# Justin-Huber/SfM-project

Hardware: AMD Instinct MI355X
Metric: verified matches/sec (match+RANSAC) (higher is better)
Workload: dtype int8 MFMA -> exact int32 (K1), f32 (K2); 1 GPU; cfg4: all 124750 unordered pairs of 500 synthetic images x 4096 128-D u8 SIFT-like descriptors; L2 match (mutual cross check + ratio 4/5) + 8-point RANSAC 4096 hyp/pair (seed 42, Sampson 1 px^2, min 15 inliers); launches of <= 131072 pairs; n_img=500, k=4096, n_hyp=4096, pairs_total=124750, pairs_rank0=124750, launches_rank0=1, parallelism=pair-sharded dp1

## Files before the change

include/sfmcore.h:

```cpp
#ifndef SFMCORE_H
#define SFMCORE_H

#include <stdint.h>

#ifdef __cplusplus
extern "C" {
#endif

#define SFM_OK 0
#define SFM_ERR_INVALID (-1)
#define SFM_ERR_HIP (-2)
#define SFM_ERR_NOMEM (-3)

#define SFM_METRIC_L2 0
#define SFM_METRIC_HAMMING 1

#define SFM_XC_NONE 0
#define SFM_XC_MUTUAL 1
#define SFM_XC_OPENCV 2

typedef struct sfm_ctx sfm_ctx;

typedef struct sfm_match_params {
    int32_t metric;
    int32_t cross_check;
    int32_t ratio_num;
    int32_t ratio_den;
    int64_t max_dist;
} sfm_match_params;

typedef struct sfm_ransac_params {
    int32_t n_hyp;
    int32_t min_inliers;
    float thr;
    int32_t _pad;
    uint64_t seed;
} sfm_ransac_params;

int sfm_ctx_create(int32_t device, sfm_ctx** out);
int sfm_ctx_destroy(sfm_ctx* ctx);
int sfm_ctx_set_stream(sfm_ctx* ctx, void* hip_stream);
int sfm_ctx_sync(sfm_ctx* ctx);
const char* sfm_last_error(void);
int32_t sfm_version(void);

int sfm_match_batch(sfm_ctx* ctx, const uint8_t* desc, const int32_t* n_kp, int32_t n_img,
                    int32_t k_max, int32_t dim, const int32_t* pairs, int32_t n_pairs,
                    const sfm_match_params* prm, int32_t* out_count, int32_t* out_match,
                    int32_t* out_dist);
int sfm_match_batch_both(sfm_ctx* ctx, const uint8_t* desc, const int32_t* n_kp, int32_t n_img,
                         int32_t k_max, int32_t dim, const int32_t* pairs, int32_t n_pairs,
                         const sfm_match_params* prm, int32_t* out_count, int32_t* out_match,
                         int32_t* out_dist);

int sfm_ransac_f_batch(sfm_ctx* ctx, const float* kps, int32_t n_img, int32_t k_max,
                       const int32_t* pairs, int32_t n_pairs, const int32_t* match_count,
                       const int32_t* matches, const sfm_ransac_params* prm,
                       int32_t* out_inl_count, int32_t* out_best_h, uint8_t* out_mask,
                       float* out_F, float* out_norm);

int sfm_ransac_f_batch_f64(sfm_ctx* ctx, const double* kps, int32_t n_img, int32_t k_max,
                           const int32_t* pairs, int32_t n_pairs, const int32_t* match_count,
                           const int32_t* matches, const sfm_ransac_params* prm,
                           int32_t* out_inl_count, int32_t* out_best_h, uint8_t* out_mask,
                           double* out_F, double* out_norm);

int sfm_ransac_counts(sfm_ctx* ctx, const float* kps, int32_t n_img, int32_t k_max,
                      const int32_t* pairs, int32_t n_pairs, const int32_t* match_count,
                      const int32_t* matches, const sfm_ransac_params* prm, int32_t* out_counts,
                      float* out_norm, float* out_hyp_F, uint8_t* out_hyp_mask);

int sfm_ransac_stats(sfm_ctx* ctx, int32_t enable, uint64_t* out);
int sfm_ransac_wave_stops(sfm_ctx* ctx, int32_t n_pairs, int32_t n_hyp, uint32_t* out);

int sfm_ransac_h_batch(sfm_ctx* ctx, const float* kps, int32_t n_img, int32_t k_max,
                       const int32_t* pairs, int32_t n_pairs, const int32_t* match_count,
                       const int32_t* matches, const sfm_ransac_params* prm,
                       int32_t* out_inl_count, int32_t* out_best_h, uint8_t* out_mask,
                       float* out_H, float* out_norm);

int sfm_ransac_h_counts(sfm_ctx* ctx, const float* kps, int32_t n_img, int32_t k_max,
                        const int32_t* pairs, int32_t n_pairs, const int32_t* match_count,
                        const int32_t* matches, const sfm_ransac_params* prm, int32_t* out_counts,
                        float* out_norm, float* out_hyp_H);

typedef struct sfm_two_view_pose_params {
    int32_t struct_size;
    int32_t min_inliers;
    float wide_key;
} sfm_two_view_pose_params;
int sfm_two_view_pose_batch(sfm_ctx* ctx, const float* kps, int32_t n_img, int32_t k_max,
                            const int32_t* pairs, int32_t n_pairs, const int32_t* match_count,
                            const int32_t* matches, const uint8_t* mask,
                            const int32_t* inl_count, const double* intr,
                            const sfm_two_view_pose_params* prm, double* out_E, double* out_R,
                            double* out_t, int32_t* out_stat, float* out_median_key);

int sfm_graph_offsets(sfm_ctx* ctx, int32_t n_pairs, const int32_t* inl_count,
                      int32_t min_inliers, int64_t* out_offsets);
int sfm_graph_rows(sfm_ctx* ctx, int32_t n_pairs, int32_t k_max, int32_t pair_base,
                   const int32_t* match_count, const int32_t* matches, const uint8_t* mask,
                   const int32_t* inl_count, int32_t min_inliers, const int64_t* offsets,
                   int32_t* out_rows);
int sfm_graph_rows_packed(sfm_ctx* ctx, int32_t n_pairs, int32_t k_max,
                          const int32_t* match_count, const int32_t* matches, const uint8_t* mask,
                          const int32_t* inl_count, int32_t min_inliers, const int64_t* offsets,
                          uint32_t* out_packed);
int sfm_graph_expand(sfm_ctx* ctx, int32_t n_pairs, int32_t pair_base, const int32_t* counts,
                     const int64_t* src_offsets, const int64_t* dst_offsets,
                     const uint32_t* packed, int32_t* out_rows);

int sfm_ba_jtj(sfm_ctx* ctx, int32_t n_cam, const double* cams, const double* pp, int32_t n_pt,
               const double* pts, int32_t n_obs, const int32_t* cam_idx, const int32_t* pt_idx,
               const double* uv, const int32_t* pt_ptr, const int32_t* cam_ptr,
               const int32_t* cam_obs, double loss_s, double* U, double* V, double* W,
               double* gc, double* gp, double* res, double* cost);

typedef struct sfm_ba_solve_params {
    double lambda;
    double tol;
    int32_t max_iter;
    int32_t poll;
    int32_t poll_first;
} sfm_ba_solve_params;
#define SFM_BA_POLL_DEFAULT 8

int sfm_ba_solve(sfm_ctx* ctx, int32_t n_cam, int32_t n_pt, int32_t n_obs,
                 const int32_t* cam_idx, const int32_t* pt_idx, const int32_t* pt_ptr,
                 const int32_t* cam_ptr, const int32_t* cam_obs, const double* U, const double* V,
                 const double* W, const double* gc, const double* gp,
                 const sfm_ba_solve_params* prm, double* dc, double* dp, double* info);
#define SFM_BA_STAGE_SETUP 0
#define SFM_BA_STAGE_SETUP_FINISH 1
#define SFM_BA_STAGE_ITER 2
#define SFM_BA_STAGE_ITER_FINISH 3
#define SFM_BA_STAGE_BACKSUB 4
#define SFM_BA_STAGE_MODEL 5
#define SFM_BA_STAGE_POLL 6
#define SFM_BA_STAGE_SCHUR 7
int sfm_ba_solve_stage(sfm_ctx* ctx, int32_t stage, int32_t k, int32_t n_cam, int32_t n_pt,
                       int32_t n_obs, const int32_t* cam_idx, const int32_t* pt_idx,
                       const int32_t* pt_ptr, const int32_t* cam_ptr, const int32_t* cam_obs,
                       const double* U, const double* V, const double* W, const double* gc,
                       const double* gp, const sfm_ba_solve_params* prm, double* comm, double* dc,
                       double* dp, double* info, int32_t* done);
int sfm_ba_fix_params(sfm_ctx* ctx, int32_t n_cam, int32_t n_obs, const int32_t* cam_idx,
                      const uint8_t* fixed, double* U, double* W, double* gc);
int sfm_ba_cost(sfm_ctx* ctx, int32_t n_cam, const double* cams, const double* pp, int32_t n_pt,
                const double* pts, int32_t n_obs, const int32_t* cam_idx, const int32_t* pt_idx,
                const double* uv, double loss_s, double* cost);
int sfm_ba_update(sfm_ctx* ctx, int32_t n_cam, const double* cams, const double* dc, int32_t n_pt,
                  const double* pts, const double* dp, double* cams_out, double* pts_out);

#define SFM_BA_MAX_CHUNKS 16
int sfm_ba_set_chunks(sfm_ctx* ctx, int32_t n_chunk, const int32_t* chunk_pt,
                      const int32_t* chunk_obs, int32_t n_total, const int32_t* cam_bounds);
int sfm_ba_chunk_tree(sfm_ctx* ctx, int32_t n_total, int64_t n, const double* parts, double* out);

int sfm_ba_set_schur(sfm_ctx* ctx, int32_t n_slot, const int32_t* slot_cam, int32_t n_seg,
                     const int32_t* seg, int32_t n_inst, const int32_t* inst, const int32_t* row_ptr,
                     int32_t n_ent, const int32_t* row_ent, int32_t n_group, const int32_t* sg_ptr,
                     const int32_t* sg, const int32_t* gk);

int sfm_tracks(sfm_ctx* ctx, int32_t n_img, const int32_t* img_base, int32_t n_pairs,
               const int32_t* pairs, int64_t n_rows, const int32_t* rows, int32_t min_len,
               int32_t* out_n_tracks, int32_t* out_track_ptr, int32_t* out_track_img,
               int32_t* out_track_kp);

int sfm_triangulate(sfm_ctx* ctx, int32_t n_cam, const double* cams, const double* pp,
                    int32_t n_pt, const int32_t* pt_ptr, const int32_t* cam_idx, const double* uv,
                    double* out_pts, double* out_stats);

typedef struct sfm_register_params {
    int32_t n_hyp;
    int32_t refine;
    double thr;
    uint64_t seed;
} sfm_register_params;

int sfm_register_batch(sfm_ctx* ctx, int32_t n_img, const int32_t* corr_ptr, const double* xy,
                       const double* X, const double* intr, const int32_t* img_id,
                       const sfm_register_params* prm, double* out_cams, int32_t* out_count,
                       int32_t* out_key, uint8_t* out_mask);

typedef struct sfm_orb_params {
    int32_t n_features;
    int32_t n_levels;
    double scale_factor;
    int32_t fast_threshold;
    int32_t _pad;
} sfm_orb_params;

int sfm_orb_batch(sfm_ctx* ctx, const uint8_t* images, int32_t n_img, int32_t H, int32_t W,
                  const sfm_orb_params* prm, float* out_kp, uint8_t* out_desc,
                  int32_t* out_count);

int sfm_calib_mfma_i8(sfm_ctx* ctx, float target_ms, double* out);

int sfm_match_cert_stats(sfm_ctx* ctx, int32_t enable, uint64_t* out);

#ifdef __cplusplus
}
#endif
#endif
```

sfm-project_amd/csrc/match_l2fr.hip:

```cpp
#include <algorithm>
#include <climits>
#include <cstdlib>

#include "l2fr_records.h"
#include "match_common.h"

namespace {

typedef int v4i __attribute__((ext_vector_type(4)));
typedef int v16i __attribute__((ext_vector_type(16)));
typedef __attribute__((address_space(3))) void lds_void;
typedef const __attribute__((address_space(1))) void gbl_void;

constexpr int D = 128;
#ifndef L2FR_WAVES
#define L2FR_WAVES 8
#endif
constexpr int WAVES = L2FR_WAVES;
constexpr int SCAN_THREADS = 64 * WAVES;
#ifndef L2FR_QT
#define L2FR_QT 4
#endif
constexpr int QT = L2FR_QT;
constexpr int QB = WAVES * QT * 32;
constexpr int SCAN_MIN_WAVES = 8 / QT;
#ifndef L2FR_CHUNK
#define L2FR_CHUNK 256
#endif
constexpr int CHUNK = L2FR_CHUNK;
constexpr int GROUP = 256;
constexpr int NT = CHUNK / 32;
constexpr int NK = D / 32;
constexpr int SLOTS = D / 16;
constexpr int PIECES = CHUNK * D / 1024 / WAVES;
constexpr int RPP = 1024 / D;
constexpr int KALIGN = CHUNK > GROUP ? CHUNK : GROUP;
constexpr int KMAX = 4096;
constexpr int PAD_INIT = -(1 << 30);
constexpr int E_VALID = l2fr::E_NONE;
static_assert(D == l2fr::REC_D && KMAX == l2fr::REC_KMAX, "l2fr_records.h is sized for D and KMAX");
typedef unsigned long long rec8;

enum : unsigned char { ST_DROP = 0, ST_CAND = 1, ST_SLOW = 2, ST_PASS = 3 };

__device__ __forceinline__ int swz(int row) { return (row >> 1) & 7; }

__device__ __forceinline__ void top2_insert(int& tb, int& ts, int x, int y) {
    const int med = max(min(tb, x), min(max(tb, x), y));
#ifndef L2FR_NO_ASM_MAX3
    int top;
    asm("v_max3_i32 %0, %1, %2, %3" : "=v"(top) : "v"(tb), "v"(x), "v"(y), "v"(med));
#else
    const int top = max(max(x, y), tb);
#endif
    ts = max(ts, med);
    tb = top;
}

__device__ __forceinline__ int dot128(const uint4* x, const uint4* y) {
    int s = 0;
#pragma unroll
    for (int k = 0; k < 8; ++k) {
        const uint4 u = x[k], v = y[k];
        s = __builtin_amdgcn_sdot4((int)u.x, (int)v.x, s, false);
        s = __builtin_amdgcn_sdot4((int)u.y, (int)v.y, s, false);
        s = __builtin_amdgcn_sdot4((int)u.z, (int)v.z, s, false);
        s = __builtin_amdgcn_sdot4((int)u.w, (int)v.w, s, false);
    }
    return s;
}

__device__ __forceinline__ void prep_one(int img, int j, const uint8_t* __restrict__ desc,
                                         const int32_t* __restrict__ n_kp, int k_max, int k_pad,
                                         int32_t* __restrict__ norm, int32_t* __restrict__ cinit,
                                         uint8_t* __restrict__ zero_row,
                                         uint4* __restrict__ desc_i8) {
    if (img == 0 && j < D) zero_row[j] = 0;
    if (j >= k_pad) return;
    int nv = 0;
    if (j < k_max) {
        const uint4* p = (const uint4*)(desc + ((size_t)img * k_max + j) * D);
        uint4* o8 = desc_i8 + ((size_t)img * k_max + j) * SLOTS;
#pragma unroll
        for (int q = 0; q < SLOTS; ++q) {
            const uint4 v = p[q];
            const uint4 x = make_uint4(v.x ^ 0x80808080u, v.y ^ 0x80808080u, v.z ^ 0x80808080u,
                                       v.w ^ 0x80808080u);
            o8[q] = x;
            nv = __builtin_amdgcn_sdot4((int)x.x, (int)x.x, nv, false);
            nv = __builtin_amdgcn_sdot4((int)x.y, (int)x.y, nv, false);
            nv = __builtin_amdgcn_sdot4((int)x.z, (int)x.z, nv, false);
            nv = __builtin_amdgcn_sdot4((int)x.w, (int)x.w, nv, false);
        }
    }
    const size_t o = (size_t)img * k_pad + j;
    norm[o] = nv;
    cinit[o] = (j < n_kp[img]) ? -((nv + 1) >> 1) : PAD_INIT;
}

constexpr int REC_R = 4;

#ifndef L2FR_UNIT
#define L2FR_UNIT 2
#endif
constexpr int UNIT = L2FR_UNIT;
__device__ void build_units(const int32_t* __restrict__ pairs, int n_pairs, int n_img,
                            const int32_t* __restrict__ n_kp, int4* __restrict__ uinfo,
                            int32_t* __restrict__ n_units, int* lds) {
    int* cur = lds;
    int* fu = lds + n_img;
    int* ru = lds + 2 * n_img + 1;
    __shared__ int ftot;
    const int tid = threadIdx.x;
    for (int i = tid; i < n_img; i += 1024) cur[i] = 0;
    __syncthreads();
    auto live = [&](int a, int b) { return n_kp[a] > 0 && n_kp[b] > 0; };
    for (int p = tid; p < n_pairs; p += 1024)
        if (live(pairs[2 * p], pairs[2 * p + 1])) atomicAdd(&cur[pairs[2 * p]], 1);
    __syncthreads();
    if (tid == 0) {
        int f = 0, r = 0;
        for (int i = 0; i < n_img; ++i) {
            const int c = cur[i];
            fu[i] = f;
            ru[i] = r;
            f += c / UNIT;
            r += (c % UNIT) != 0;
            cur[i] = 0;
        }
        fu[n_img] = f;
        ru[n_img] = r;
        ftot = f;
        *n_units = f + r;
    }
    __syncthreads();
    for (int t = tid; t < ru[n_img] * UNIT; t += 1024) uinfo[(size_t)ftot * UNIT + t] = make_int4(-1, 0, 0, 0);
    __syncthreads();
    for (int p = tid; p < n_pairs; p += 1024) {
        const int a = pairs[2 * p], b = pairs[2 * p + 1];
        if (!live(a, b)) continue;
        const int k = atomicAdd(&cur[a], 1);
        const int nf = UNIT * (fu[a + 1] - fu[a]);
        const int u = k < nf ? fu[a] + k / UNIT : ftot + ru[a];
        const int jj = k < nf ? k % UNIT : k - nf;
        uinfo[(size_t)u * UNIT + jj] = jj ? make_int4(p, b, n_kp[b], 0)
                                          : make_int4(p, a, b, n_kp[a] | (n_kp[b] << 16));
    }
}

__device__ void order_block(int ob, const int32_t* __restrict__ pairs, int n_pairs, int n_img,
                            int32_t* __restrict__ order_f, int32_t* __restrict__ order_r,
                            int2* __restrict__ rng, int32_t* __restrict__ n_rng,
                            const int32_t* __restrict__ n_kp, int4* __restrict__ rinfo,
                            int4* __restrict__ sinfo_f, int unit_blk, int4* __restrict__ uinfo,
                            int32_t* __restrict__ n_units, int* hist) {
    if (ob == unit_blk) {
        build_units(pairs, n_pairs, n_img, n_kp, uinfo, n_units, hist);
        return;
    }
    const int tid = threadIdx.x, col = ob == 0 ? 1 : 0;
    int32_t* order = ob == 0 ? order_f : order_r;
    for (int i = tid; i < n_img; i += 1024) hist[i] = 0;
    __syncthreads();
    for (int p = tid; p < n_pairs; p += 1024) atomicAdd(&hist[pairs[2 * p + col]], 1);
    __syncthreads();
    int* roff = hist + n_img;
    if (tid == 0) {
        int off = 0, nr = 0;
        for (int i = 0; i < n_img; ++i) {
            const int c = hist[i];
            roff[i] = nr;
            nr += (c + REC_R - 1) / REC_R;
            hist[i] = off;
            off += c;
        }
        if (ob == 0) *n_rng = nr;
    }
    __syncthreads();
    if (ob == 0)
        for (int i = tid; i < n_img; i += 1024) {
            const int c = (i + 1 < n_img ? hist[i + 1] : n_pairs) - hist[i];
            for (int k = 0; k < c; k += REC_R)
                rng[roff[i] + k / REC_R] = make_int2(hist[i] + k, min(REC_R, c - k));
        }
    __syncthreads();
    __syncthreads();
    for (int p = tid; p < n_pairs; p += 1024) {
        const int a = pairs[2 * p], b = pairs[2 * p + 1];
        const int slot = atomicAdd(&hist[col ? b : a], 1);
        order[slot] = p;
        if (ob == 0) sinfo_f[slot] = make_int4(p, a, b, n_kp[a] | (n_kp[b] << 16));
    }
    if (ob != 0) return;
    __threadfence_block();
    __syncthreads();
    const int nr = *n_rng;
    for (int r = tid; r < nr; r += 1024) {
        const int2 g = rng[r];
#pragma unroll
        for (int e = 0; e < REC_R; ++e) {
            int4 v = make_int4(-1, 0, 0, 0);
            if (e < g.y) {
                const int p = order[g.x + e], a = pairs[2 * p], b = pairs[2 * p + 1];
                v = make_int4(p, a, b, n_kp[a] | (n_kp[b] << 16));
            }
            rinfo[(size_t)r * REC_R + e] = v;
        }
    }
}

__global__ __launch_bounds__(1024) void l2fr_setup_kernel(
    int n_prep, int bpi, const uint8_t* __restrict__ desc, const int32_t* __restrict__ n_kp,
    int k_max, int k_pad, int32_t* __restrict__ norm, int32_t* __restrict__ cinit,
    uint8_t* __restrict__ zero_row, uint4* __restrict__ desc_i8, const int32_t* __restrict__ pairs,
    int n_pairs, int n_img, int32_t* __restrict__ order_f, int32_t* __restrict__ order_r,
    int2* __restrict__ rng, int32_t* __restrict__ n_rng, int4* __restrict__ rinfo,
    int4* __restrict__ sinfo_f, int unit_blk, int4* __restrict__ uinfo,
    int32_t* __restrict__ n_units) {
    extern __shared__ int hist[];
    const int b = (int)blockIdx.x;
    if (b < n_prep) {
        const int img = b / bpi;
        prep_one(img, (b - img * bpi) * 1024 + (int)threadIdx.x, desc, n_kp, k_max, k_pad, norm,
                 cinit, zero_row, desc_i8);
        return;
    }
    order_block(b - n_prep, pairs, n_pairs, n_img, order_f, order_r, rng, n_rng, n_kp, rinfo,
                sinfo_f, unit_blk, uinfo, n_units, hist);
}

__device__ __forceinline__ unsigned char classify(int e1, int e2, long long A, int rnum, int rden,
                                                  long long max_dist) {
    const long long d1lo = max(A - 2LL * e1 - 1, 0LL);
    const long long d2hi = e2 > E_VALID ? A - 2LL * e2 : sfm::DIST_INF;
    if (!sfm::ratio_ok(d1lo, d2hi, rnum, rden, true) || (max_dist >= 0 && !(d1lo < max_dist)))
        return ST_DROP;
    return (e2 == e1) ? ST_SLOW : ST_CAND;
}

struct FwdCls {
    const int32_t* norm;
    int rnum, rden;
    long long max_dist;
    rec8* fwd;
    uint8_t* cls;
};

#ifdef L2FR_CLOCK
constexpr int L2FR_CLOCK_SLOTS = 1 << 16;
constexpr int L2FR_CLOCK_W = 24;
__device__ unsigned long long g_l2fr_clock[L2FR_CLOCK_W * L2FR_CLOCK_SLOTS];
#define L2FR_STAMP(i, v) \
    if (!REV && tid == 0 && blockIdx.x < L2FR_CLOCK_SLOTS) g_l2fr_clock[L2FR_CLOCK_W * (size_t)blockIdx.x + (i)] = (v)
#else
#define L2FR_STAMP(i, v)
#endif

template <bool REV>
__global__ __launch_bounds__(SCAN_THREADS, SCAN_MIN_WAVES) void l2fr_scan_kernel(
    const uint8_t* __restrict__ desc, const int32_t* __restrict__ n_kp, int k_max, int k_pad,
    const int32_t* __restrict__ cinit, const uint8_t* __restrict__ zero_row,
    const int32_t* __restrict__ pairs, int n_qblk, const int32_t* __restrict__ pair_order,
    const int4* __restrict__ sinfo, int n_blk, const int4* __restrict__ qlist,
    const int32_t* __restrict__ qcount, int4* __restrict__ out, FwdCls fc,
    const int32_t* __restrict__ n_units) {
    __shared__ __attribute__((aligned(16))) unsigned char lds0[CHUNK * D + CHUNK * 4];
    __shared__ __attribute__((aligned(16))) unsigned char lds1[CHUNK * D + CHUNK * 4];

    int p, qi, ti, nq, nb, qb;
    int p2 = -1, ti2 = 0, nb2 = 0;
    int pos = 0, kk = 0;
    if (!REV && n_units) {
        const int nu = *n_units;
        const int u8 = (nu + 7) >> 3;
        const int l = (int)(blockIdx.x >> 3);
        qb = u8 > 0 ? l / u8 : n_qblk;
        pos = (l - qb * u8) * 8 + (int)(blockIdx.x & 7);
        if (qb >= n_qblk || pos >= nu) return;
        const int4 u = sinfo[(size_t)UNIT * pos];
        asm volatile("" : : "s"(u.x), "s"(u.y), "s"(u.z), "s"(u.w));
        p = u.x;
        qi = u.y;
        ti = u.z;
        nq = u.w & 0xFFFF;
        nb = u.w >> 16;
    } else {
        const int ppx = (int)(gridDim.x >> 3) / n_qblk;
        const int l = (int)(blockIdx.x >> 3);
        const int pos = (int)(blockIdx.x & 7) * ppx + l % ppx;
        qb = l / ppx;
        if (pos >= n_blk) return;
        if (REV) {
            p = pair_order[pos];
            qi = pairs[2 * p + 1];
            ti = pairs[2 * p];
            nq = qcount[p];
            nb = n_kp[ti];
        } else {
            const int4 u = sinfo[pos];
            asm volatile("" : : "s"(u.x), "s"(u.y), "s"(u.z), "s"(u.w));
            p = u.x;
            qi = u.y;
            ti = u.z;
            nq = u.w & 0xFFFF;
            nb = u.w >> 16;
        }
    }
    if (qb * QB >= nq || nb <= 0) return;
    const int tid = threadIdx.x, wave = tid >> 6, lane = tid & 63, h = lane >> 5, r32 = lane & 31;
    L2FR_STAMP(0, __builtin_amdgcn_s_memrealtime());

    const uint8_t* db = desc + (size_t)ti * k_max * D;
    const int32_t* cib = cinit + (size_t)ti * k_pad;
    int n_chunk = (nb + CHUNK - 1) / CHUNK;
    const uint8_t* db2 = desc;
    const int32_t* cib2 = cinit;
    auto find_next = [&]() {
        p2 = -1;
        if (REV || !n_units || ++kk >= UNIT) return;
        const int4 v = sinfo[(size_t)UNIT * pos + kk];
        p2 = v.x;
        ti2 = v.y;
        nb2 = v.z;
        db2 = desc + (size_t)ti2 * k_max * D;
        cib2 = cinit + (size_t)ti2 * k_pad;
    };
    find_next();

    auto stage = [&](const uint8_t* sdb, const int32_t* scib, int snb, int ch, unsigned char* dst) {
#pragma unroll
        for (int i = 0; i < PIECES; ++i) {
            const int piece = wave * PIECES + i;
            const int row = piece * RPP + lane / SLOTS;
            const int slot = (lane % SLOTS) ^ swz(row);
            const int j = ch * CHUNK + row;
            const uint8_t* src = (j < snb) ? sdb + (size_t)j * D + slot * 16 : zero_row + slot * 16;
            __builtin_amdgcn_global_load_lds((gbl_void*)src, (lds_void*)(dst + piece * 1024), 16, 0, 0);
        }
        if (tid < CHUNK / 4) {
            const int32_t* src = scib + ch * CHUNK + tid * 4;
            __builtin_amdgcn_global_load_lds((gbl_void*)src, (lds_void*)(dst + CHUNK * D + wave * 1024),
                                             16, 0, 0);
        }
    };
    auto stage_next = [&](int ch, unsigned char* dst) {
        if (ch + 1 < n_chunk) stage(db, cib, nb, ch + 1, dst);
        else if (p2 >= 0) stage(db2, cib2, nb2, 0, dst);
    };

    const int qbase = qb * QB + wave * QT * 32;
    const bool active = qbase < nq;
    const uint8_t* da = desc + (size_t)qi * k_max * D;

    auto emit = [&](int e, int e1, int e2, int t) {
        if (REV) {
            out[(size_t)p * k_pad + e] = make_int4(e1, e2, t, 0);
        } else {
            fc.fwd[(size_t)p * k_pad + e] = l2fr::pack_fwd(e1, e2, t);
            const unsigned char st =
                classify(e1, e2, fc.norm[(size_t)qi * k_pad + e], fc.rnum, fc.rden, fc.max_dist);
            fc.cls[(size_t)p * k_pad + e] =
                st == ST_CAND ? (uint8_t)t : (st == ST_SLOW ? l2fr::CLS_SLOW : l2fr::CLS_DROP);
        }
    };

#if L2FR_MFMA16
    constexpr int QS = 2 * QT;
    const int g4 = lane >> 4, r16 = lane & 15;
    v4i bq[QS][2];
    int tb[QS], ts[QS], t1[QS];
#pragma unroll
    for (int c = 0; c < QS; ++c) {
        const int e = qbase + c * 16 + r16;
        int row = -1;
        if (e < nq) row = REV ? qlist[(size_t)p * k_pad + e].y : e;
        const v4i* src = (const v4i*)((row >= 0) ? da + (size_t)row * D + 32 * g4 : zero_row + 32 * g4);
        bq[c][0] = src[0];
        bq[c][1] = src[1];
        tb[c] = INT_MIN; ts[c] = INT_MIN; t1[c] = 0;
    }
    v4i acc[QS][2];
    auto process = [&](int ch, const unsigned char* cur, unsigned char* nxt) __attribute__((always_inline)) {
        stage_next(ch, nxt);
        const int nt = min(NT, (nb - ch * CHUNK + 31) >> 5);
        if (active) {
            const int* Ci = (const int*)(cur + CHUNK * D);
            auto load_tile = [&](int tt, v4i (&af)[2][2], v4i (&init)[2]) {
#pragma unroll
                for (int u = 0; u < 2; ++u) {
                    const int row = tt * 32 + 16 * u + r16;
                    const int sw = swz(row);
#pragma unroll
                    for (int s = 0; s < 2; ++s)
#ifdef L2FR_ABL_NOLDS
                        af[u][s] = bq[(tt + u + s) & (QS - 1)][s];
#else
                        af[u][s] = *(const v4i*)(cur + row * D + (((2 * g4 + s) ^ sw) << 4));
#endif
#ifdef L2FR_ABL_NOLDS
                    init[u] = v4i{tt, u, tt, u};
#else
                    init[u] = *(const v4i*)(Ci + tt * 32 + 16 * u + 4 * g4);
#endif
                }
            };
            v4i af[2][2], init[2];
            load_tile(0, af, init);
            for (int tt = 0; tt < nt; ++tt) {
                const int gt = ch * NT + tt;
#ifndef L2FR_NO_MPRIO
                __builtin_amdgcn_s_setprio(1);
#endif
#pragma unroll
                for (int s = 0; s < 2; ++s)
#pragma unroll
                    for (int u = 0; u < 2; ++u)
#pragma unroll
                        for (int c = 0; c < QS; ++c)
                            acc[c][u] = __builtin_amdgcn_mfma_i32_16x16x64_i8(
                                af[u][s], bq[c][s], s == 0 ? init[u] : acc[c][u], 0, 0, 0);
#ifndef L2FR_NO_MPRIO
                __builtin_amdgcn_s_setprio(0);
#endif
                if (tt + 1 < nt) load_tile(tt + 1, af, init);
#pragma unroll
                for (int c = 0; c < QS; ++c) {
                    const int o = tb[c];
#ifdef L2FR_ABL_NOEPI
                    tb[c] = max(tb[c], acc[c][0][0] ^ acc[c][1][3]);
#else
#pragma unroll
                    for (int u = 0; u < 2; ++u) {
                        top2_insert(tb[c], ts[c], acc[c][u][0], acc[c][u][1]);
                        top2_insert(tb[c], ts[c], acc[c][u][2], acc[c][u][3]);
                    }
#endif
                    t1[c] = (tb[c] != o) ? gt : t1[c];
                }
            }
        }
    };
#else
    v4i bq[QT][NK];
    int tb[QT], ts[QT], t1[QT];
#pragma unroll
    for (int c = 0; c < QT; ++c) {
        const int e = qbase + c * 32 + r32;
        int row = -1;
        if (e < nq) row = REV ? qlist[(size_t)p * k_pad + e].y : e;
        const v4i* src = (const v4i*)((row >= 0) ? da + (size_t)row * D + (D / 2) * h
                                                 : zero_row + (D / 2) * h);
#pragma unroll
        for (int s = 0; s < NK; ++s) bq[c][s] = src[s];
        tb[c] = INT_MIN; ts[c] = INT_MIN; t1[c] = 0;
    }

    v16i acc[QT];
    auto epi_all = [&](int gt) {
#pragma unroll
        for (int u = 0; u < QT; ++u) {
            const int o = tb[u];
#ifdef L2FR_ABL_NOEPI
            tb[u] = max(tb[u], acc[u][0] ^ acc[u][15]);
#else
#pragma unroll
            for (int r = 0; r < 16; r += 2) top2_insert(tb[u], ts[u], acc[u][r], acc[u][r + 1]);
#endif
            t1[u] = (tb[u] != o) ? gt : t1[u];
        }
    };

    auto process = [&](int ch, const unsigned char* cur, unsigned char* nxt) __attribute__((always_inline)) {
        stage_next(ch, nxt);
        const int nt = min(NT, (nb - ch * CHUNK + 31) >> 5);
        if (active) {
            const int* Ci = (const int*)(cur + CHUNK * D);
            auto load_tile = [&](int tt, v4i (&af)[NK], v16i& init) {
                const int row = tt * 32 + r32;
                const int sw = swz(row);
#pragma unroll
                for (int s = 0; s < NK; ++s)
#ifdef L2FR_ABL_NOLDS
                    af[s] = bq[(tt + s) & (QT - 1)][s];
#else
                    af[s] = *(const v4i*)(cur + row * D + ((((SLOTS / 2) * h + s) ^ sw) << 4));
#endif
#pragma unroll
                for (int g = 0; g < 4; ++g) {
#ifdef L2FR_ABL_NOLDS
                    const v4i cv = v4i{tt, g, tt, g};
#else
                    const v4i cv = *(const v4i*)(Ci + tt * 32 + 8 * g + 4 * h);
#endif
                    init[4 * g + 0] = cv.x; init[4 * g + 1] = cv.y;
                    init[4 * g + 2] = cv.z; init[4 * g + 3] = cv.w;
                }
            };
            v4i af[NK];
            v16i init;
            load_tile(0, af, init);
            for (int tt = 0; tt < nt; ++tt) {
                const int gt = ch * NT + tt;
#ifndef L2FR_NO_MPRIO
                __builtin_amdgcn_s_setprio(1);
#endif
#pragma unroll
                for (int s = 0; s < NK; ++s)
#pragma unroll
                    for (int c = 0; c < QT; ++c)
                        acc[c] = __builtin_amdgcn_mfma_i32_32x32x32_i8(af[s], bq[c][s],
                                                                        s == 0 ? init : acc[c], 0, 0, 0);
#ifndef L2FR_NO_MPRIO
                __builtin_amdgcn_s_setprio(0);
#endif
                if (tt + 1 < nt) load_tile(tt + 1, af, init);
                epi_all(gt);
            }
        }
    };
#endif

    auto epilogue = [&]() {
#if L2FR_MFMA16
#pragma unroll
        for (int c = 0; c < QS; ++c) {
            int e1 = tb[c], e2 = ts[c], t = t1[c];
#pragma unroll
            for (int m = 16; m <= 32; m <<= 1) {
                const int P1 = __shfl_xor(e1, m), P2 = __shfl_xor(e2, m), PT = __shfl_xor(t, m);
                e2 = max(min(e1, P1), max(e2, P2));
                t = e1 > P1 ? t : (P1 > e1 ? PT : min(t, PT));
                e1 = max(e1, P1);
            }
            const int e = qbase + c * 16 + r16;
            if (g4 == 0 && e < nq) emit(e, e1, e2, t);
            tb[c] = INT_MIN; ts[c] = INT_MIN; t1[c] = 0;
        }
#else
#pragma unroll
        for (int c = 0; c < QT; ++c) {
            const int P1 = __shfl_xor(tb[c], 32), P2 = __shfl_xor(ts[c], 32),
                      PT = __shfl_xor(t1[c], 32);
            const int e1 = max(tb[c], P1);
            const int e2 = max(min(tb[c], P1), max(ts[c], P2));
            const int t = tb[c] > P1 ? t1[c] : (P1 > tb[c] ? PT : min(t1[c], PT));
            const int e = qbase + c * 32 + r32;
            if (h == 0 && e < nq) emit(e, e1, e2, t);
            tb[c] = INT_MIN; ts[c] = INT_MIN; t1[c] = 0;
        }
#endif
    };

    if (n_chunk > 0) stage(db, cib, nb, 0, lds0);
    __syncthreads();
    L2FR_STAMP(1, __builtin_amdgcn_s_memrealtime());
    L2FR_STAMP(2, __builtin_amdgcn_s_memtime());
    auto run_pair = [&](unsigned char* s0, unsigned char* s1) __attribute__((always_inline)) {
        for (int ch = 0; ch < n_chunk; ch += 2) {
            process(ch, s0, s1);
            __syncthreads();
            if (ch < 16) L2FR_STAMP(3 + ch, __builtin_amdgcn_s_memrealtime());
            if (ch + 1 < n_chunk) process(ch + 1, s1, s0);
            __syncthreads();
            if (ch + 1 < 16) L2FR_STAMP(4 + ch, __builtin_amdgcn_s_memrealtime());
        }
    };
    int g = 0;
    for (;;) {
        if (g & 1)
            run_pair(lds1, lds0);
        else
            run_pair(lds0, lds1);
        g += n_chunk;
        L2FR_STAMP(19, __builtin_amdgcn_s_memtime());
        L2FR_STAMP(20, __builtin_amdgcn_s_memrealtime());
        if (active) epilogue();
        if (p2 < 0) break;
        p = p2;
        ti = ti2;
        nb = nb2;
        db = db2;
        cib = cib2;
        n_chunk = (nb + CHUNK - 1) / CHUNK;
        find_next();
    }
#ifdef L2FR_CLOCK
    L2FR_STAMP(21, __builtin_amdgcn_s_memrealtime());
    L2FR_STAMP(22, (unsigned)__builtin_amdgcn_s_getreg((31 << 11) | 4));
    L2FR_STAMP(23, (unsigned)__builtin_amdgcn_s_getreg((15 << 11) | 20));
#endif
}

struct Top2 { long long b1; int j1; long long b2; };

__device__ __forceinline__ Top2 top2_merge(Top2 x, Top2 y) {
    const bool xf = (x.b1 < y.b1) || (x.b1 == y.b1 && x.j1 < y.j1);
    Top2 r;
    r.b1 = xf ? x.b1 : y.b1;
    r.j1 = xf ? x.j1 : y.j1;
    r.b2 = min(min(x.b2, y.b2), xf ? y.b1 : x.b1);
    return r;
}

__device__ Top2 exact_row_scan(const uint4* qrow, const uint8_t* db, const int32_t* normb, int nb,
                               int qnorm, Top2* red) {
    const int tid = threadIdx.x;
    uint4 x[SLOTS];
#pragma unroll
    for (int s = 0; s < SLOTS; ++s) x[s] = qrow[s];
    Top2 m{sfm::DIST_INF, INT_MAX, sfm::DIST_INF};
    for (int j = tid; j < nb; j += 256) {
        const int dot = dot128(x, (const uint4*)(db + (size_t)j * D));
        const long long d = (long long)qnorm + normb[j] - 2LL * dot;
        m = top2_merge(m, Top2{d, j, sfm::DIST_INF});
    }
    red[tid] = m;
    __syncthreads();
    for (int s = 128; s > 0; s >>= 1) {
        if (tid < s) red[tid] = top2_merge(red[tid], red[tid + s]);
        __syncthreads();
    }
    const Top2 r = red[0];
    __syncthreads();
    return r;
}

__device__ __forceinline__ int compact_rec(bool keep, int4 rec, int base, int* wsum, int4* dst) {
    const int tid = threadIdx.x, lane = tid & 63, wave = tid >> 6;
    const unsigned long long bal = __ballot(keep);
    const int pre = __popcll(bal & ((1ull << lane) - 1ull));
    if (lane == 0) wsum[wave] = __popcll(bal);
    __syncthreads();
    int off = 0, tot = 0;
    for (int w = 0; w < 4; ++w) {
        const int s = wsum[w];
        off += (w < wave) ? s : 0;
        tot += s;
    }
    if (keep) dst[base + off + pre] = rec;
    __syncthreads();
    return base + tot;
}

#ifndef L2FR_REC_SB
#define L2FR_REC_SB 2
#endif
constexpr int REC_SB = L2FR_REC_SB;
__global__ __launch_bounds__(256, REC_SB > 2 ? 2 : 3) void l2fr_recover_mfma_kernel(
    const uint8_t* __restrict__ desc, int k_max, int k_pad, const int32_t* __restrict__ norm,
    const int32_t* __restrict__ cinit, const int4* __restrict__ rinfo,
    const int32_t* __restrict__ n_rng, const rec8* __restrict__ fwd,
    const uint8_t* __restrict__ cls, int rnum, int rden, long long max_dist,
    rec8* __restrict__ qst) {
    __shared__ unsigned short clist[REC_R * KMAX];
    __shared__ __attribute__((aligned(16))) int gini[GROUP];
    __shared__ unsigned char gpar[GROUP];
    __shared__ unsigned long long wlo[4], whi[4];
    __shared__ int toff[9];
    const int ngrp = k_pad / GROUP;
    const int ri = (int)(blockIdx.x / ngrp), grp = (int)(blockIdx.x % ngrp), tid = threadIdx.x;
    if (ri >= *n_rng) return;
    const int wave = tid >> 6, lane = tid & 63, h = lane >> 5, r32 = lane & 31;
    int4 pi[REC_R];
#pragma unroll
    for (int e = 0; e < REC_R; ++e) pi[e] = rinfo[(size_t)ri * REC_R + e];
    const int b = pi[0].z, nb = pi[0].w >> 16;
    const int ntiles = (nb + 31) >> 5, tg = grp * 8;
    if (nb <= 0 || tg >= ntiles) return;
    const uint8_t* db = desc + (size_t)b * k_max * D;

    uint4 cv[REC_R];
#pragma unroll
    for (int e = 0; e < REC_R; ++e) {
        cv[e] = make_uint4(0xFFFFFFFFu, 0xFFFFFFFFu, 0xFFFFFFFFu, 0xFFFFFFFFu);
        if (pi[e].x >= 0 && tid * 16 < (pi[e].w & 0xFFFF))
            cv[e] = ((const uint4*)(cls + (size_t)pi[e].x * k_pad))[tid];
    }
    v4i af[2][NK];
#pragma unroll
    for (int u = 0; u < 2; ++u) {
        const int row = (tg + 2 * wave + u) * 32 + r32;
#pragma unroll
        for (int s = 0; s < NK; ++s)
            af[u][s] = row < nb ? *(const v4i*)(db + (size_t)row * D + 64 * h + 16 * s) : v4i{0, 0, 0, 0};
    }
    {
        const size_t o = (size_t)b * k_pad + tg * 32 + tid;
        gini[tid] = cinit[o];
        gpar[tid] = (unsigned char)(norm[o] & 1);
    }
    unsigned msk[REC_R];
    unsigned long long lo = 0, hi = 0;
    const unsigned g8 = 0x01010101u * ((unsigned)grp << 3);
#pragma unroll
    for (int e = 0; e < REC_R; ++e) {
        const int na = pi[e].x >= 0 ? (pi[e].w & 0xFFFF) : 0;
        const unsigned cw[4] = {cv[e].x, cv[e].y, cv[e].z, cv[e].w};
        unsigned m = 0;
#pragma unroll
        for (int k = 0; k < 4; ++k) {
            const unsigned t = (cw[k] ^ g8) & 0xF8F8F8F8u;
            const unsigned nz = ((t & 0x7F7F7F7Fu) + 0x7F7F7F7Fu) | t;
            const unsigned z = ~nz & 0x80808080u;
            m |= (((z >> 7) & 1u) | ((z >> 14) & 2u) | ((z >> 21) & 4u) | ((z >> 28) & 8u)) << (4 * k);
        }
        const int lim = na - tid * 16;
        m &= lim >= 16 ? 0xFFFFu : (lim <= 0 ? 0u : (1u << lim) - 1u);
        msk[e] = m;
        for (unsigned mm = m; mm; mm &= mm - 1) {
            const int k = __builtin_ctz(mm);
            const unsigned c = (cw[k >> 2] >> (8 * (k & 3))) & 7u;
            const unsigned long long one = 1ull << (16 * (c & 3));
            if (c & 4) hi += one; else lo += one;
        }
    }
    unsigned long long plo = lo, phi = hi;
#pragma unroll
    for (int d = 1; d < 64; d <<= 1) {
        const unsigned long long vl = __shfl_up(plo, d), vh = __shfl_up(phi, d);
        if (lane >= d) { plo += vl; phi += vh; }
    }
    if (lane == 63) { wlo[wave] = plo; whi[wave] = phi; }
    __syncthreads();
    unsigned long long blo = 0, bhi = 0, tlo = 0, thi = 0;
#pragma unroll
    for (int w = 0; w < 4; ++w) {
        blo += w < wave ? wlo[w] : 0ull;
        bhi += w < wave ? whi[w] : 0ull;
        tlo += wlo[w];
        thi += whi[w];
    }
    unsigned long long slo = 0, shi = 0;
    {
        int o = 0;
#pragma unroll
        for (int t = 0; t < 8; ++t) {
            const unsigned long long tot = t < 4 ? tlo : thi, bef = t < 4 ? blo : bhi,
                                     mine = t < 4 ? plo - lo : phi - hi;
            const int sh = 16 * (t & 3);
            const unsigned long long v =
                (unsigned long long)(o + (int)((bef >> sh) & 0xFFFF) + (int)((mine >> sh) & 0xFFFF)) << sh;
            if (t < 4) slo |= v; else shi |= v;
            if (tid == 0) toff[t] = o;
            o += (int)((tot >> sh) & 0xFFFF);
        }
        if (tid == 0) toff[8] = o;
    }
#pragma unroll
    for (int e = 0; e < REC_R; ++e) {
        const unsigned cw[4] = {cv[e].x, cv[e].y, cv[e].z, cv[e].w};
        for (unsigned mm = msk[e]; mm; mm &= mm - 1) {
            const int k = __builtin_ctz(mm);
            const unsigned c = (cw[k >> 2] >> (8 * (k & 3))) & 7u;
            const int sh = 16 * (c & 3);
            const unsigned long long cur = (c & 4) ? shi : slo, inc = 1ull << sh;
            clist[(int)((cur >> sh) & 0xFFFF)] = (unsigned short)((e << 12) | (tid * 16 + k));
            if (c & 4) shi += inc; else slo += inc;
        }
    }
    __syncthreads();
    const int w0 = toff[2 * wave], w1 = toff[2 * wave + 2];
    const int t0 = tg + 2 * wave;
    for (int c0 = w0; c0 < w1; c0 += 32 * REC_SB) {
        v4i bf[REC_SB][NK];
        rec8 rc[REC_SB];
        int ce[REC_SB], AA[REC_SB];
#pragma unroll
        for (int k = 0; k < REC_SB; ++k) {
            const int c = c0 + 32 * k + r32;
            ce[k] = -1;
            if (c < w1) {
                const int en = clist[c], e = en >> 12, q = en & 0xFFF;
                int p = pi[0].x, a = pi[0].y;
#pragma unroll
                for (int f = 1; f < REC_R; ++f) {
                    p = e == f ? pi[f].x : p;
                    a = e == f ? pi[f].y : a;
                }
                const uint8_t* xr = desc + ((size_t)a * k_max + q) * D + 64 * h;
#pragma unroll
                for (int s = 0; s < NK; ++s) bf[k][s] = *(const v4i*)(xr + 16 * s);
                rc[k] = fwd[(size_t)p * k_pad + q];
                AA[k] = norm[(size_t)a * k_pad + q];
                ce[k] = en;
            } else {
#pragma unroll
                for (int s = 0; s < NK; ++s) bf[k][s] = v4i{0, 0, 0, 0};
                rc[k] = 0;
            }
        }
#pragma unroll
        for (int k = 0; k < REC_SB; ++k) {
            if (c0 + 32 * k >= w1) break;
            const l2fr::Fwd r = l2fr::unpack_fwd(rc[k]);
            const int mine = r.tile - t0;
            int hit = -1;
#pragma unroll
            for (int u = 0; u < 2; ++u) {
                v16i acc;
                const int* gi = gini + (2 * wave + u) * 32 + 4 * h;
#pragma unroll
                for (int g = 0; g < 4; ++g) {
                    const v4i c4 = *(const v4i*)(gi + 8 * g);
                    acc[4 * g + 0] = c4.x; acc[4 * g + 1] = c4.y;
                    acc[4 * g + 2] = c4.z; acc[4 * g + 3] = c4.w;
                }
#pragma unroll
                for (int s = 0; s < NK; ++s)
                    acc = __builtin_amdgcn_mfma_i32_32x32x32_i8(af[u][s], bf[k][s], acc, 0, 0, 0);
#pragma unroll
                for (int rr = 0; rr < 16; ++rr)
                    hit = (mine == u && acc[rr] == r.e1) ? 8 * (rr >> 2) + 4 * h + (rr & 3) : hit;
            }
            hit = max(hit, __shfl_xor(hit, 32));
            if (h == 0 && ce[k] >= 0) {
                const int e = ce[k] >> 12;
                int p = pi[0].x;
#pragma unroll
                for (int f = 1; f < REC_R; ++f) p = e == f ? pi[f].x : p;
                rec8* qs = qst + (size_t)p * k_pad + (ce[k] & 0xFFF);
                if (hit < 0) {
                    *qs = l2fr::pack_res(ST_SLOW, 0, 0, 0);
                } else {
                    const int jg = (2 * wave + mine) * 32 + hit;
                    const long long A = AA[k];
                    const long long d1 = A - 2LL * r.e1 - gpar[jg];
                    const long long d2lo = r.e2 > E_VALID ? A - 2LL * r.e2 - 1 : sfm::DIST_INF;
                    const long long d2hi = r.e2 > E_VALID ? A - 2LL * r.e2 : sfm::DIST_INF;
                    int st;
                    if (max_dist >= 0 && !(d1 < max_dist)) st = ST_DROP;
                    else if (sfm::ratio_ok(d1, d2lo, rnum, rden, true)) st = ST_PASS;
                    else if (!sfm::ratio_ok(d1, d2hi, rnum, rden, true)) st = ST_DROP;
                    else st = ST_SLOW;
                    *qs = l2fr::pack_res(st, tg * 32 + jg, (int)d1, 1);
                }
            }
        }
    }
}

__global__ __launch_bounds__(256) void l2fr_compact_kernel(
    const uint8_t* __restrict__ desc, const int32_t* __restrict__ n_kp, int k_max, int k_pad,
    const int32_t* __restrict__ norm, const int32_t* __restrict__ pairs,
    const uint8_t* __restrict__ cls, rec8* __restrict__ qst, int rnum, int rden, long long max_dist,
    int4* __restrict__ surv, int32_t* __restrict__ scount, int32_t* __restrict__ smax,
    int32_t* __restrict__ out_count, int32_t* __restrict__ out_match,
    int32_t* __restrict__ out_dist) {
    __shared__ Top2 red[256];
    __shared__ int slow[256];
    __shared__ int nslow, wsum[8], wmax[4];
    const int p = blockIdx.x, tid = threadIdx.x;
    const int a = pairs[2 * p], b = pairs[2 * p + 1];
    const int na = n_kp[a], nb = n_kp[b];
    const bool direct = out_count != nullptr;
    int32_t* om = direct ? out_match + (size_t)p * k_max * 2 : nullptr;
    int32_t* od = direct ? out_dist + (size_t)p * k_max : nullptr;
    if (na <= 0 || nb <= 0) {
        if (tid == 0) {
            if (direct) out_count[p] = 0;
            else scount[p] = 0;
        }
        return;
    }
    rec8* qs = qst + (size_t)p * k_pad;
    const uint8_t* cl = cls + (size_t)p * k_pad;
    const int32_t* na_norm = norm + (size_t)a * k_pad;
    const int32_t* nb_norm = norm + (size_t)b * k_pad;
    const uint4* qa = (const uint4*)(desc + (size_t)a * k_max * D);
    const uint8_t* db = desc + (size_t)b * k_max * D;
    int4* sv = surv + (size_t)p * k_pad;
    int base = 0, dmax = 0;
    for (int q0 = 0; q0 < na; q0 += 256) {
        const int q = q0 + tid;
        int4 r = make_int4(ST_DROP, 0, 0, 0);
        if (q < na) {
            const unsigned char c = cl[q];
            const rec8 raw = qs[q];
            if (c == l2fr::CLS_SLOW) {
                r.x = ST_SLOW;
            } else if (c != l2fr::CLS_DROP) {
                const l2fr::Res u = l2fr::unpack_res(raw);
                r = make_int4(u.st, u.j1, u.d1, u.exact);
            }
        }
        if (tid == 0) nslow = 0;
        __syncthreads();
        if (r.x == ST_SLOW) slow[atomicAdd(&nslow, 1)] = tid;
        __syncthreads();
        const int ns = nslow;
        for (int i = 0; i < ns; ++i) {
            const int who = slow[i], qq = q0 + who;
            const Top2 e = exact_row_scan(qa + (size_t)qq * SLOTS, db, nb_norm, nb, na_norm[qq], red);
            if (tid == who) {
                bool keep = sfm::ratio_ok(e.b1, e.b2, rnum, rden, true);
                keep = keep && (max_dist < 0 || e.b1 < max_dist);
                r = make_int4(keep ? ST_PASS : ST_DROP, e.j1, (int)e.b1, 1);
                if (!direct) qs[qq] = l2fr::pack_res(r.x, r.y, r.z, 1);
            }
        }
        const bool keep = r.x == ST_PASS;
        dmax = keep ? max(dmax, r.z) : dmax;
        if (direct)
            base = sfm::compact256(keep, q, r.y, r.z, base, wsum, om, od);
        else
            base = compact_rec(keep, make_int4(q, r.y, r.z, 0), base, wsum, sv);
    }
    if (tid == 0) {
        if (direct) out_count[p] = base;
        else scount[p] = base;
    }
    if (direct) return;
#pragma unroll
    for (int m = 32; m > 0; m >>= 1) dmax = max(dmax, __shfl_xor(dmax, m));
    if ((tid & 63) == 0) wmax[tid >> 6] = dmax;
    __syncthreads();
    if (tid == 0) smax[p] = max(max(wmax[0], wmax[1]), max(wmax[2], wmax[3]));
}

constexpr int CERT_TMAX = 2048;
constexpr long long CERT_CAP_DEFAULT = 16384;

__global__ __launch_bounds__(256) void l2fr_mutual_cert_kernel(
    const uint8_t* __restrict__ desc, const int32_t* __restrict__ n_kp, int k_max, int k_pad,
    const int32_t* __restrict__ norm, const int32_t* __restrict__ pairs,
    const rec8* __restrict__ fwd, const uint8_t* __restrict__ cls, const rec8* __restrict__ qst,
    const int4* __restrict__ surv, const int32_t* __restrict__ scount,
    const int32_t* __restrict__ smax, long long cap, int32_t* __restrict__ rcount,
    uint8_t* __restrict__ flag, unsigned long long* __restrict__ stats,
    int32_t* __restrict__ out_count, int32_t* __restrict__ out_match,
    int32_t* __restrict__ out_dist) {
    __shared__ unsigned long long owner[KMAX];
    __shared__ int tbound[CERT_TMAX];
    __shared__ unsigned short tq[CERT_TMAX];
    __shared__ unsigned char killed[KMAX];
    __shared__ int wsum[8];
    __shared__ int nthreat;
    const int p = blockIdx.x, tid = threadIdx.x;
    const int a = pairs[2 * p], b = pairs[2 * p + 1];
    const int na = n_kp[a], nb = n_kp[b];
    const int S = (na > 0 && nb > 0) ? scount[p] : 0;
    if (cap <= 0) {
        if (tid == 0) {
            rcount[p] = S;
            flag[p] = 1;
            if (stats) atomicAdd(&stats[1], 1ull);
        }
        return;
    }
    if (S == 0) {
        if (tid == 0) {
            rcount[p] = 0;
            flag[p] = 0;
            out_count[p] = 0;
            if (stats) atomicAdd(&stats[0], 1ull);
        }
        return;
    }
    const rec8* fw = fwd + (size_t)p * k_pad;
    const rec8* qs = qst + (size_t)p * k_pad;
    const uint8_t* cl = cls + (size_t)p * k_pad;
    const int4* sv = surv + (size_t)p * k_pad;
    const int32_t* na_norm = norm + (size_t)a * k_pad;
    const int32_t* nb_norm = norm + (size_t)b * k_pad;
    const uint4* qa = (const uint4*)(desc + (size_t)a * k_max * D);
    const uint4* dbv = (const uint4*)(desc + (size_t)b * k_max * D);

    const long long T = smax[p];
    for (int k = tid; k < S; k += 256) killed[k] = 0;
    for (int j = tid; j < nb; j += 256) owner[j] = ~0ull;
    if (tid == 0) nthreat = 0;
    __syncthreads();

    for (int q = tid; q < na; q += 256) {
        const unsigned char c = cl[q];
        const rec8 raw = qs[q];
        l2fr::Res r{ST_DROP, 0, 0, 0};
        if (c != l2fr::CLS_DROP) r = l2fr::unpack_res(raw);
        const l2fr::Fwd f = l2fr::unpack_fwd(fw[q]);
        const long long A = na_norm[q];
        long long bound;
        if (r.exact == 1) {
            if ((unsigned)r.j1 < (unsigned)nb)
                atomicMin(&owner[r.j1], ((unsigned long long)(unsigned)r.d1 << 32) | (unsigned)q);
            bound = f.e2 > E_VALID ? A - 2LL * f.e2 - 1 : sfm::DIST_INF;
        } else {
            bound = A - 2LL * f.e1 - 1;
        }
        if (bound <= T) {
            const int i = atomicAdd(&nthreat, 1);
            if (i < CERT_TMAX) {
                tq[i] = (unsigned short)q;
                tbound[i] = (int)bound;
            }
        }
    }
    __syncthreads();
    const int nT = nthreat;
    if (nT > CERT_TMAX || (long long)nT * S > cap) {
        if (tid == 0) {
            rcount[p] = S;
            flag[p] = 1;
            if (stats) atomicAdd(&stats[1], 1ull);
        }
        return;
    }
    unsigned dots = 0;
    for (int i = tid; i < nT * S; i += 256) {
        const int t = i / S, k = i - t * S;
        const int4 s = sv[k];
        const int qp = tq[t];
        if (qp == s.x || s.z < tbound[t]) continue;
        const int dot = dot128(qa + (size_t)qp * SLOTS, dbv + (size_t)s.y * SLOTS);
        const long long d = (long long)na_norm[qp] + nb_norm[s.y] - 2LL * dot;
        if (d < s.z || (d == s.z && qp < s.x)) killed[k] = 1;
        ++dots;
    }
    if (stats && dots) atomicAdd(&stats[2], (unsigned long long)dots);
    __syncthreads();
    int32_t* om = out_match + (size_t)p * k_max * 2;
    int32_t* od = out_dist + (size_t)p * k_max;
    int base = 0;
    for (int k0 = 0; k0 < S; k0 += 256) {
        const int k = k0 + tid;
        int4 s = make_int4(0, 0, 0, 0);
        bool keep = false;
        if (k < S) {
            s = sv[k];
            keep = !killed[k] &&
                   owner[s.y] == (((unsigned long long)(unsigned)s.z << 32) | (unsigned)s.x);
        }
        base = sfm::compact256(keep, s.x, s.y, s.z, base, wsum, om, od);
    }
    if (tid == 0) {
        out_count[p] = base;
        rcount[p] = 0;
        flag[p] = 0;
        if (stats) atomicAdd(&stats[0], 1ull);
    }
}

__global__ __launch_bounds__(256) void l2fr_final_kernel(
    const uint8_t* __restrict__ desc, const int32_t* __restrict__ n_kp, int k_max, int k_pad,
    const int32_t* __restrict__ norm, const int32_t* __restrict__ cinit,
    const int32_t* __restrict__ pairs, const int4* __restrict__ surv,
    const int32_t* __restrict__ scount, const int4* __restrict__ rev, int mutual,
    const uint8_t* __restrict__ flag, int32_t* __restrict__ out_count,
    int32_t* __restrict__ out_match, int32_t* __restrict__ out_dist) {
    __shared__ int wsum[8];
    __shared__ int amb[256];
    __shared__ int namb;
    __shared__ unsigned char keepx[256];
    __shared__ long long redd[256];
    __shared__ int redq[256];
    const int p = blockIdx.x, tid = threadIdx.x;
    if (flag && !flag[p]) return;
    const int a = pairs[2 * p], b = pairs[2 * p + 1];
    const int na = n_kp[a], nb = n_kp[b];
    const int S = (na > 0 && nb > 0) ? scount[p] : 0;
    const int4* sv = surv + (size_t)p * k_pad;
    const int4* rv = rev + (size_t)p * k_pad;
    const int32_t* na_norm = norm + (size_t)a * k_pad;
    const int32_t* nb_norm = norm + (size_t)b * k_pad;
    const int32_t* ca = cinit + (size_t)a * k_pad;
    const uint8_t* da = desc + (size_t)a * k_max * D;
    const uint4* dbv = (const uint4*)(desc + (size_t)b * k_max * D);
    int32_t* om = out_match + (size_t)p * k_max * 2;
    int32_t* od = out_dist + (size_t)p * k_max;
    int base = 0;
    for (int k0 = 0; k0 < S; k0 += 256) {
        const int k = k0 + tid;
        int4 s = make_int4(0, 0, 0, 0);
        bool keep = false;
        if (tid == 0) namb = 0;
        __syncthreads();
        if (k < S) {
            s = sv[k];
            keep = true;
            if (mutual) {
                const int4 r = rv[k];
                const int dot = (int)(((long long)na_norm[s.x] + nb_norm[s.y] - s.z) >> 1);
                const int ep = dot + ca[s.x];
                keep = (ep == r.x) && (r.y < r.x);
                if (ep == r.x && r.y == r.x) amb[atomicAdd(&namb, 1)] = tid;
            }
        }
        keepx[tid] = keep;
        __syncthreads();
        const int nam = namb;
        for (int i = 0; i < nam; ++i) {
            const int who = amb[i];
            const int4 e = sv[k0 + who];
            uint4 y[SLOTS];
#pragma unroll
            for (int u = 0; u < SLOTS; ++u) y[u] = dbv[(size_t)e.y * SLOTS + u];
            long long bd = sfm::DIST_INF;
            int bq = INT_MAX;
            for (int q = tid; q < na; q += 256) {
                const int dot = dot128((const uint4*)(da + (size_t)q * D), y);
                const long long d = (long long)na_norm[q] + nb_norm[e.y] - 2LL * dot;
                if (d < bd) { bd = d; bq = q; }
            }
            redd[tid] = bd; redq[tid] = bq;
            __syncthreads();
            for (int st = 128; st > 0; st >>= 1) {
                if (tid < st) {
                    const long long od2 = redd[tid + st];
                    const int oq = redq[tid + st];
                    if (od2 < redd[tid] || (od2 == redd[tid] && oq < redq[tid])) {
                        redd[tid] = od2; redq[tid] = oq;
                    }
                }
                __syncthreads();
            }
            if (tid == 0) keepx[who] = (redq[0] == e.x);
            __syncthreads();
        }
        keep = keepx[tid] != 0 && k < S;
        base = sfm::compact256(keep, s.x, s.y, s.z, base, wsum, om, od);
    }
    if (tid == 0) out_count[p] = base;
}

__global__ void l2fr_dump_kernel(const int32_t* __restrict__ n_kp, const int32_t* __restrict__ pairs,
                                 int k_max, int k_pad, const int4* __restrict__ rec,
                                 const rec8* __restrict__ fwd8,
                                 const int32_t* __restrict__ cnt, int32_t* __restrict__ out_count,
                                 int32_t* __restrict__ out_match, int32_t* __restrict__ out_dist) {
    const int p = blockIdx.x;
    const int n = cnt ? cnt[p] : n_kp[pairs[2 * p]];
    for (int i = threadIdx.x; i < n; i += blockDim.x) {
        int4 r;
        if (rec) {
            r = rec[(size_t)p * k_pad + i];
        } else {
            const l2fr::Fwd f = l2fr::unpack_fwd(fwd8[(size_t)p * k_pad + i]);
            r = make_int4(f.e1, f.e2, f.tile, 0);
        }
        out_match[((size_t)p * k_max + i) * 2] = r.x;
        out_match[((size_t)p * k_max + i) * 2 + 1] = r.y;
        out_dist[(size_t)p * k_max + i] = r.z;
    }
    if (threadIdx.x == 0) out_count[p] = n;
}

}

int sfm_match_l2fr_launch(sfm_ctx* ctx, const uint8_t* desc, const int32_t* n_kp, int32_t n_img,
                          int32_t k_max, const int32_t* pairs, int32_t n_pairs,
                          const sfm_match_params* prm, int32_t* out_count, int32_t* out_match,
                          int32_t* out_dist) {
    hipStream_t st = ctx->stream;
    if (k_max == 0) {
        SFM_HIP_CHECK(hipMemsetAsync(out_count, 0, sizeof(int32_t) * n_pairs, st));
        return SFM_OK;
    }
    const int k_pad = (int)sfm::align_up((size_t)k_max, KALIGN);
    SFM_REQUIRE(k_pad <= KMAX, "sfm_match_batch: L2 matcher needs k_max <= 4096");
    const int n_qblk = (k_max + QB - 1) / QB;
    const size_t tab = (size_t)n_img * k_pad * sizeof(int32_t);
    const size_t recb = (size_t)n_pairs * k_pad * sizeof(int4);
    const size_t cntb = sfm::align_up(sizeof(int32_t) * (size_t)n_pairs, 256);
    const size_t descb = sfm::align_up((size_t)n_img * k_max * D, 256);
    const size_t ordb = sfm::align_up(sizeof(int32_t) * (size_t)n_pairs, 256);
    const size_t clsb = sfm::align_up((size_t)n_pairs * k_pad, 256);
    const int n_rng_max = n_pairs / REC_R + n_img + 1;
    const size_t rngb = sfm::align_up(sizeof(int2) * (size_t)n_rng_max, 256);
    const size_t rinfob = sizeof(int4) * (size_t)n_rng_max * REC_R;
    const size_t sinfob = sfm::align_up(sizeof(int4) * (size_t)n_pairs, 256);
    const size_t uinfob = sfm::align_up(UNIT * sizeof(int4) * (size_t)n_pairs, 256);
    const size_t flagb = sfm::align_up((size_t)n_pairs, 256);
    char* ws = (char*)sfm::workspace(ctx, 256 + 2 * tab + 2 * recb + cntb + descb + 2 * ordb + clsb +
                                              256 + rngb + rinfob + 256 + sinfob + uinfob + 256 +
                                              cntb + flagb + cntb);
    if (!ws) return SFM_ERR_NOMEM;
    char* w = ws;
    uint8_t* zero_row = (uint8_t*)w; w += 256;
    int32_t* norm = (int32_t*)w; w += tab;
    int32_t* cinit = (int32_t*)w; w += tab;
    int4* surv = (int4*)w; w += recb;
    int4* rev = (int4*)w; w += recb;
    rec8* fwd = (rec8*)rev;
    rec8* qst = fwd + (size_t)n_pairs * k_pad;
    int32_t* scount = (int32_t*)w; w += cntb;
    uint8_t* desc_i8 = (uint8_t*)w; w += descb;
    int32_t* ord_f = (int32_t*)w; w += ordb;
    int32_t* ord_r = (int32_t*)w; w += ordb;
    uint8_t* cls = (uint8_t*)w; w += clsb;
    int32_t* n_rng = (int32_t*)w; w += 256;
    int2* rng = (int2*)w; w += rngb;
    int4* rinfo = (int4*)w; w += rinfob;
    int4* sinfo_f = (int4*)sfm::align_up((size_t)w, 256);
    int4* uinfo = (int4*)((char*)sinfo_f + sinfob);
    int32_t* n_units = (int32_t*)((char*)uinfo + uinfob);
    int32_t* rcount = (int32_t*)((char*)n_units + 256);
    uint8_t* flag = (uint8_t*)rcount + cntb;
    int32_t* smax = (int32_t*)(flag + flagb);
    static const bool units_env = [] {
        const char* e = getenv("SFM_L2FR_UNITS");
        return !(e && e[0] == '0');
    }();
    const bool units = units_env && (3 * (size_t)n_img + 2) * sizeof(int) <= 65536;
    const int ppx = (n_pairs + 7) / 8;
    const int n_blk = n_pairs;
    const int grid = 8 * ppx * n_qblk;
    const bool mutual = prm->cross_check == SFM_XC_MUTUAL;

    const int32_t* sord_f = ord_f;
    const int32_t* sord_r = ord_r;
    const int unit_blk = units ? (mutual ? 2 : 1) : -1;
    const int bpi = (k_pad + 1023) / 1024, n_prep = bpi * n_img;
    hipLaunchKernelGGL(l2fr_setup_kernel, dim3(n_prep + (mutual ? 2 : 1) + (units ? 1 : 0)),
                       dim3(1024), ((units ? 3 : 2) * (size_t)n_img + 2) * sizeof(int), st, n_prep,
                       bpi, desc, n_kp, k_max, k_pad, norm, cinit, zero_row, (uint4*)desc_i8, pairs,
                       n_pairs, n_img, ord_f, ord_r, rng, n_rng, rinfo, sinfo_f, unit_blk, uinfo,
                       n_units);
    SFM_HIP_CHECK(hipGetLastError());
    const FwdCls fc{norm, prm->ratio_num, prm->ratio_den, (long long)prm->max_dist, fwd, cls};
    hipLaunchKernelGGL(l2fr_scan_kernel<false>, dim3(grid), dim3(SCAN_THREADS), 0, st, desc_i8, n_kp, k_max,
                       k_pad, cinit, zero_row, pairs, n_qblk, sord_f,
                       (const int4*)(units ? uinfo : sinfo_f), n_blk, (const int4*)nullptr,
                       (const int32_t*)nullptr, (int4*)nullptr, fc,
                       (const int32_t*)(units ? n_units : nullptr));
    SFM_HIP_CHECK(hipGetLastError());
    const char* dbg = getenv("SFM_L2FR_DEBUG");
    const int dmode = dbg ? atoi(dbg) : 0;
    if (dmode == 1) {
        hipLaunchKernelGGL(l2fr_dump_kernel, dim3(n_pairs), dim3(256), 0, st, n_kp, pairs, k_max,
                           k_pad, (const int4*)nullptr, (const rec8*)fwd, (const int32_t*)nullptr,
                           out_count, out_match, out_dist);
        return SFM_OK;
    }
    hipLaunchKernelGGL(l2fr_recover_mfma_kernel, dim3(n_rng_max * (k_pad / GROUP)), dim3(256), 0, st,
                       desc_i8, k_max, k_pad, norm, cinit, (const int4*)rinfo, (const int32_t*)n_rng,
                       (const rec8*)fwd, (const uint8_t*)cls, prm->ratio_num, prm->ratio_den,
                       (long long)prm->max_dist, qst);
    SFM_HIP_CHECK(hipGetLastError());
    const bool direct = !mutual && dmode == 0;
    hipLaunchKernelGGL(l2fr_compact_kernel, dim3(n_pairs), dim3(256), 0, st, desc_i8, n_kp, k_max,
                       k_pad, norm, pairs, (const uint8_t*)cls, qst, prm->ratio_num, prm->ratio_den,
                       (long long)prm->max_dist, surv, scount, smax,
                       direct ? out_count : nullptr,
                       out_match, out_dist);
    SFM_HIP_CHECK(hipGetLastError());
    if (direct) return SFM_OK;
    if (dmode == 2) {
        hipLaunchKernelGGL(l2fr_dump_kernel, dim3(n_pairs), dim3(256), 0, st, n_kp, pairs, k_max,
                           k_pad, (const int4*)surv, (const rec8*)nullptr, (const int32_t*)scount,
                           out_count, out_match, out_dist);
        return SFM_OK;
    }
    const char* ce = getenv("SFM_L2FR_CERT");
    const bool cert = mutual && dmode == 0 && !(ce && ce[0] == '0');
    if (cert) {
        const char* cc = getenv("SFM_L2FR_CERT_CAP");
        const long long cap = cc ? atoll(cc) : CERT_CAP_DEFAULT;
        unsigned long long* stats = ctx->cert_stats ? ctx->cert_acc : nullptr;
        if (stats)
            SFM_HIP_CHECK(hipMemsetAsync(stats, 0, 3 * sizeof(unsigned long long), st));
        hipLaunchKernelGGL(l2fr_mutual_cert_kernel, dim3(n_pairs), dim3(256), 0, st, desc_i8, n_kp,
                           k_max, k_pad, norm, pairs, (const rec8*)fwd, (const uint8_t*)cls,
                           (const rec8*)qst, (const int4*)surv, (const int32_t*)scount,
                           (const int32_t*)smax, cap, rcount, flag, stats,
                           out_count, out_match, out_dist);
        SFM_HIP_CHECK(hipGetLastError());
    }
    if (mutual) {
        hipLaunchKernelGGL(l2fr_scan_kernel<true>, dim3(grid), dim3(SCAN_THREADS), 0, st, desc_i8, n_kp,
                           k_max, k_pad, cinit, zero_row, pairs, n_qblk, sord_r,
                           (const int4*)nullptr, n_blk,
                           (const int4*)surv, (const int32_t*)(cert ? rcount : scount), rev, fc,
                           (const int32_t*)nullptr);
        SFM_HIP_CHECK(hipGetLastError());
    }
    if (dmode == 3) {
        hipLaunchKernelGGL(l2fr_dump_kernel, dim3(n_pairs), dim3(256), 0, st, n_kp, pairs, k_max,
                           k_pad, (const int4*)rev, (const rec8*)nullptr, (const int32_t*)scount,
                           out_count, out_match, out_dist);
        return SFM_OK;
    }
    hipLaunchKernelGGL(l2fr_final_kernel, dim3(n_pairs), dim3(256), 0, st, desc_i8, n_kp, k_max,
                       k_pad, norm, cinit, pairs, surv, scount, rev, mutual ? 1 : 0,
                       (const uint8_t*)(cert ? flag : nullptr), out_count, out_match, out_dist);
    SFM_HIP_CHECK(hipGetLastError());
    return SFM_OK;
}

extern "C" int sfm_match_cert_stats(sfm_ctx* ctx, int32_t enable, uint64_t* out) {
    SFM_REQUIRE(ctx, "sfm_match_cert_stats: ctx is NULL");
    SFM_HIP_CHECK(hipSetDevice(ctx->device));
    if (!ctx->cert_acc) {
        SFM_HIP_CHECK(hipMalloc(&ctx->cert_acc, 3 * sizeof(unsigned long long)));
        SFM_HIP_CHECK(hipMemsetAsync(ctx->cert_acc, 0, 3 * sizeof(unsigned long long), ctx->stream));
    }
    if (out) {
        unsigned long long h[3];
        SFM_HIP_CHECK(hipMemcpyAsync(h, ctx->cert_acc, sizeof(h), hipMemcpyDeviceToHost, ctx->stream));
        SFM_HIP_CHECK(hipStreamSynchronize(ctx->stream));
        out[0] = h[0]; out[1] = h[1]; out[2] = h[2];
    }
    ctx->cert_stats = enable ? 1 : 0;
    return SFM_OK;
}

#ifdef L2FR_CLOCK
extern "C" int sfm_debug_l2fr_stamps(unsigned long long* host, int32_t n_blocks) {
    const size_t n = L2FR_CLOCK_W * (size_t)std::min(n_blocks, L2FR_CLOCK_SLOTS);
    SFM_HIP_CHECK(hipDeviceSynchronize());
    SFM_HIP_CHECK(hipMemcpyFromSymbol(host, HIP_SYMBOL(g_l2fr_clock), n * sizeof(unsigned long long)));
    return SFM_OK;
}
#endif
```

sfm-project_amd/sfmcore.py:

```python
from __future__ import annotations

import ctypes as C
import os
import threading

import numpy as np

_HERE = os.path.dirname(os.path.abspath(__file__))
LIB_PATH = os.environ.get("SFMCORE_LIB") or os.path.join(_HERE, "lib", "libsfmcore.so")

METRIC_L2, METRIC_HAMMING = 0, 1
XC_NONE, XC_MUTUAL, XC_OPENCV = 0, 1, 2

EXPORTED = ["sfm_ctx_create", "sfm_ctx_destroy", "sfm_ctx_set_stream", "sfm_ctx_sync",
            "sfm_last_error", "sfm_version", "sfm_match_batch", "sfm_ransac_f_batch",
            "sfm_ba_jtj", "sfm_graph_offsets", "sfm_graph_rows", "sfm_ba_solve", "sfm_ba_cost",
            "sfm_ba_update", "sfm_tracks", "sfm_triangulate", "sfm_register_batch",
            "sfm_ba_fix_params", "sfm_orb_batch", "sfm_ransac_counts", "sfm_ba_solve_stage",
            "sfm_ransac_stats", "sfm_ransac_f_batch_f64", "sfm_graph_rows_packed",
            "sfm_graph_expand", "sfm_match_batch_both", "sfm_ransac_wave_stops",
            "sfm_ba_set_chunks", "sfm_ba_chunk_tree", "sfm_ba_set_schur", "sfm_calib_mfma_i8",
            "sfm_match_cert_stats", "sfm_ransac_h_batch", "sfm_ransac_h_counts",
            "sfm_two_view_pose_batch"]


class SfmCoreError(RuntimeError):
    pass


class MatchParams(C.Structure):
    _fields_ = [("metric", C.c_int32), ("cross_check", C.c_int32), ("ratio_num", C.c_int32),
                ("ratio_den", C.c_int32), ("max_dist", C.c_int64)]


class BaSolveParams(C.Structure):
    _fields_ = [("lam", C.c_double), ("tol", C.c_double), ("max_iter", C.c_int32),
                ("poll", C.c_int32), ("poll_first", C.c_int32)]


class RegisterParams(C.Structure):
    _fields_ = [("n_hyp", C.c_int32), ("refine", C.c_int32), ("thr", C.c_double),
                ("seed", C.c_uint64)]


class OrbParams(C.Structure):
    _fields_ = [("n_features", C.c_int32), ("n_levels", C.c_int32), ("scale_factor", C.c_double),
                ("fast_threshold", C.c_int32), ("_pad", C.c_int32)]


class RansacParams(C.Structure):
    _fields_ = [("n_hyp", C.c_int32), ("min_inliers", C.c_int32), ("thr", C.c_float),
                ("_pad", C.c_int32), ("seed", C.c_uint64)]


class TwoViewPoseParams(C.Structure):
    _fields_ = [("struct_size", C.c_int32), ("min_inliers", C.c_int32), ("wide_key", C.c_float)]


(BA_STAGE_SETUP, BA_STAGE_SETUP_FINISH, BA_STAGE_ITER, BA_STAGE_ITER_FINISH, BA_STAGE_BACKSUB,
 BA_STAGE_MODEL, BA_STAGE_POLL, BA_STAGE_SCHUR) = range(8)
BA_FINISH_VEC_MAX_CAM = 1024

_lib = None
_lock = threading.Lock()


def load_library(path: str = LIB_PATH):
    global _lib
    with _lock:
        if _lib is not None:
            return _lib
        import torch
        if not os.path.exists(path):
            if os.path.exists("/opt/rocm/bin/hipcc"):
                from build_lib import build
                build()
            if not os.path.exists(path):
                raise SfmCoreError(f"libsfmcore.so not found at {path}; run __graft_entry__.build()")
        L = C.CDLL(path)
        vp, i32, i64, f64 = C.c_void_p, C.c_int32, C.c_int64, C.c_double
        L.sfm_ctx_create.argtypes = [i32, C.POINTER(vp)]
        L.sfm_ctx_destroy.argtypes = [vp]
        L.sfm_ctx_set_stream.argtypes = [vp, vp]
        L.sfm_ctx_sync.argtypes = [vp]
        L.sfm_last_error.restype = C.c_char_p
        L.sfm_version.restype = i32
        L.sfm_match_batch.argtypes = [vp, vp, vp, i32, i32, i32, vp, i32, C.POINTER(MatchParams),
                                      vp, vp, vp]
        L.sfm_match_batch_both.argtypes = L.sfm_match_batch.argtypes
        L.sfm_ransac_f_batch.argtypes = [vp, vp, i32, i32, vp, i32, vp, vp,
                                         C.POINTER(RansacParams), vp, vp, vp, vp, vp]
        L.sfm_ransac_f_batch_f64.argtypes = L.sfm_ransac_f_batch.argtypes
        L.sfm_ransac_counts.argtypes = [vp, vp, i32, i32, vp, i32, vp, vp,
                                        C.POINTER(RansacParams), vp, vp, vp, vp]
        L.sfm_ransac_h_batch.argtypes = L.sfm_ransac_f_batch.argtypes
        L.sfm_ransac_h_counts.argtypes = [vp, vp, i32, i32, vp, i32, vp, vp,
                                          C.POINTER(RansacParams), vp, vp, vp]
        L.sfm_two_view_pose_batch.argtypes = [vp, vp, i32, i32, vp, i32, vp, vp, vp, vp, vp,
                                              C.POINTER(TwoViewPoseParams), vp, vp, vp, vp, vp]
        L.sfm_ransac_stats.argtypes = [vp, i32, vp]
        L.sfm_ransac_wave_stops.argtypes = [vp, i32, i32, vp]
        L.sfm_match_cert_stats.argtypes = [vp, i32, vp]
        L.sfm_calib_mfma_i8.argtypes = [vp, C.c_float, vp]
        L.sfm_ba_jtj.argtypes = [vp, i32, vp, vp, i32, vp, i32, vp, vp, vp, vp, vp, vp, f64, vp,
                                 vp, vp, vp, vp, vp, vp]
        L.sfm_ba_solve.argtypes = [vp, i32, i32, i32, vp, vp, vp, vp, vp, vp, vp, vp, vp, vp,
                                   C.POINTER(BaSolveParams), vp, vp, vp]
        L.sfm_ba_solve_stage.argtypes = [vp, i32, i32, i32, i32, i32, vp, vp, vp, vp, vp, vp, vp,
                                         vp, vp, vp, C.POINTER(BaSolveParams), vp, vp, vp, vp, vp]
        L.sfm_ba_cost.argtypes = [vp, i32, vp, vp, i32, vp, i32, vp, vp, vp, f64, vp]
        L.sfm_ba_update.argtypes = [vp, i32, vp, vp, i32, vp, vp, vp, vp]
        L.sfm_ba_fix_params.argtypes = [vp, i32, i32, vp, vp, vp, vp, vp]
        L.sfm_ba_set_chunks.argtypes = [vp, i32, vp, vp, i32, vp]
        L.sfm_ba_set_schur.argtypes = [vp, i32, vp, i32, vp, i32, vp, vp, i32, vp, i32, vp, vp, vp]
        L.sfm_ba_chunk_tree.argtypes = [vp, i32, i64, vp, vp]
        L.sfm_orb_batch.argtypes = [vp, vp, i32, i32, i32, C.POINTER(OrbParams), vp, vp, vp]
        L.sfm_register_batch.argtypes = [vp, i32, vp, vp, vp, vp, vp, C.POINTER(RegisterParams),
                                         vp, vp, vp, vp]
        L.sfm_triangulate.argtypes = [vp, i32, vp, vp, i32, vp, vp, vp, vp, vp]
        L.sfm_tracks.argtypes = [vp, i32, vp, i32, vp, i64, vp, i32, vp, vp, vp, vp]
        L.sfm_graph_offsets.argtypes = [vp, i32, vp, i32, vp]
        L.sfm_graph_rows.argtypes = [vp, i32, i32, i32, vp, vp, vp, vp, i32, vp, vp]
        L.sfm_graph_rows_packed.argtypes = [vp, i32, i32, vp, vp, vp, vp, i32, vp, vp]
        L.sfm_graph_expand.argtypes = [vp, i32, i32, vp, vp, vp, vp, vp]
        for name in EXPORTED:
            getattr(L, name).restype = getattr(L, name).restype or C.c_int
        _lib = L
        return L


def angle_key(angle_deg) -> np.float32:
    return np.float32(np.sin(np.deg2rad(float(angle_deg))) ** 2)


def _check(rc: int):
    if rc != 0:
        msg = load_library().sfm_last_error().decode(errors="replace")
        raise SfmCoreError(f"libsfmcore error {rc}: {msg}")


def _ptr(t) -> int:
    return t.data_ptr()


def _expect(fn: str, *specs):
    for name, t, dt, tail in specs:
        ok = t.dtype == dt and t.is_cuda and t.is_contiguous()
        ok = ok and tuple(t.shape[t.dim() - len(tail):]) == tuple(tail) and t.dim() == len(tail) + 1
        if not ok:
            raise SfmCoreError(f"{fn}: {name} must be a contiguous device {dt} tensor of shape "
                               f"[n, {', '.join(map(str, tail))}]" if tail else
                               f"{fn}: {name} must be a contiguous device {dt} vector")


class Context:

    def __init__(self, device: int = 0):
        import torch
        self.torch = torch
        if not torch.cuda.is_available():
            raise SfmCoreError("no HIP device visible: the sfm core has no CPU fallback")
        self.lib = load_library()
        self.device = device
        h = C.c_void_p()
        _check(self.lib.sfm_ctx_create(device, C.byref(h)))
        self.handle = h
        self._stream = None

    def close(self):
        if getattr(self, "handle", None):
            self.lib.sfm_ctx_destroy(self.handle)
            self.handle = None

    def __del__(self):
        try:
            self.close()
        except Exception:
            pass

    def _bind_stream(self):
        s = self.torch.cuda.current_stream(self.device).cuda_stream
        if s != self._stream:
            _check(self.lib.sfm_ctx_set_stream(self.handle, C.c_void_p(s)))
            self._stream = s

    def sync(self):
        _check(self.lib.sfm_ctx_sync(self.handle))

    def match_batch(self, desc, n_kp, pairs, metric=METRIC_L2, cross_check=XC_MUTUAL,
                    ratio=None, max_dist=-1, out=None):
        torch = self.torch
        n_img, k_max, dim = desc.shape
        P = pairs.shape[0]
        for t, dt in ((desc, torch.uint8), (n_kp, torch.int32), (pairs, torch.int32)):
            if t.dtype != dt or not t.is_cuda or not t.is_contiguous():
                raise SfmCoreError("match_batch: expected contiguous device tensors "
                                   "(desc u8, n_kp i32, pairs i32)")
        dev = desc.device
        if out is None:
            out = (torch.empty(P, dtype=torch.int32, device=dev),
                   torch.empty((P, k_max, 2), dtype=torch.int32, device=dev),
                   torch.empty((P, k_max), dtype=torch.int32, device=dev))
        num, den = (0, 0) if ratio is None else ratio
        prm = MatchParams(metric, cross_check, int(num), int(den), int(max_dist))
        self._bind_stream()
        _check(self.lib.sfm_match_batch(self.handle, _ptr(desc), _ptr(n_kp), n_img, k_max, dim,
                                        _ptr(pairs), P, C.byref(prm), _ptr(out[0]), _ptr(out[1]),
                                        _ptr(out[2])))
        return out

    def match_batch_both(self, desc, n_kp, pairs, metric=METRIC_HAMMING, cross_check=XC_OPENCV,
                         max_dist=-1, out=None):
        torch = self.torch
        n_img, k_max, dim = desc.shape
        P = pairs.shape[0]
        for t, dt in ((desc, torch.uint8), (n_kp, torch.int32), (pairs, torch.int32)):
            if t.dtype != dt or not t.is_cuda or not t.is_contiguous():
                raise SfmCoreError("match_batch_both: expected contiguous device tensors "
                                   "(desc u8, n_kp i32, pairs i32)")
        dev = desc.device
        if out is None:
            out = (torch.empty(2 * P, dtype=torch.int32, device=dev),
                   torch.empty((2 * P, k_max, 2), dtype=torch.int32, device=dev),
                   torch.empty((2 * P, k_max), dtype=torch.int32, device=dev))
        prm = MatchParams(metric, cross_check, 0, 0, int(max_dist))
        self._bind_stream()
        _check(self.lib.sfm_match_batch_both(self.handle, _ptr(desc), _ptr(n_kp), n_img, k_max,
                                             dim, _ptr(pairs), P, C.byref(prm), _ptr(out[0]),
                                             _ptr(out[1]), _ptr(out[2])))
        return out

    def orb_batch(self, images, n_features=500, n_levels=8, scale_factor=1.2, fast_threshold=20,
                  out=None):
        torch = self.torch
        if images.dtype != torch.uint8 or not images.is_cuda or not images.is_contiguous():
            raise SfmCoreError("orb_batch: expected a contiguous u8 device tensor [n_img,H,W]")
        n_img, H, W = images.shape
        dev = images.device
        if out is None:
            out = (torch.empty((n_img, n_features, 6), dtype=torch.float32, device=dev),
                   torch.empty((n_img, n_features, 32), dtype=torch.uint8, device=dev),
                   torch.empty(n_img, dtype=torch.int32, device=dev))
        prm = OrbParams(int(n_features), int(n_levels), float(scale_factor), int(fast_threshold), 0)
        self._bind_stream()
        _check(self.lib.sfm_orb_batch(self.handle, _ptr(images), n_img, H, W, C.byref(prm),
                                      _ptr(out[0]), _ptr(out[1]), _ptr(out[2])))
        return out

    def ransac_batch(self, kps, pairs, count, match, n_hyp=4096, seed=42, thr=1.0,
                     min_inliers=15, out=None):
        torch = self.torch
        n_img, k_max, _ = kps.shape
        P = pairs.shape[0]
        dev = kps.device
        if kps.dtype not in (torch.float32, torch.float64) or not kps.is_contiguous():
            raise SfmCoreError("ransac_batch: kps must be contiguous float32 or float64")
        f64 = kps.dtype == torch.float64
        if out is None:
            out = dict(inl_count=torch.empty(P, dtype=torch.int32, device=dev),
                       best_h=torch.empty(P, dtype=torch.int32, device=dev),
                       mask=torch.empty((P, k_max), dtype=torch.uint8, device=dev),
                       F=torch.empty((P, 9), dtype=kps.dtype, device=dev),
                       norm=torch.empty((P, 6), dtype=kps.dtype, device=dev))
        prm = RansacParams(int(n_hyp), int(min_inliers), float(thr), 0, int(seed))
        self._bind_stream()
        fn = self.lib.sfm_ransac_f_batch_f64 if f64 else self.lib.sfm_ransac_f_batch
        _check(fn(self.handle, _ptr(kps), n_img, k_max, _ptr(pairs), P,
                                           _ptr(count), _ptr(match), C.byref(prm),
                                           _ptr(out["inl_count"]), _ptr(out["best_h"]),
                                           _ptr(out["mask"]), _ptr(out["F"]), _ptr(out["norm"])))
        return out

    def ransac_counts(self, kps, pairs, count, match, n_hyp=4096, seed=42, thr=1.0,
                      hyp_F=False, hyp_mask=False):
        torch = self.torch
        n_img, k_max, _ = kps.shape
        P = pairs.shape[0]
        dev = kps.device
        if kps.dtype != torch.float32 or not kps.is_contiguous():
            raise SfmCoreError("ransac_counts: kps must be contiguous float32")
        counts = torch.empty((P, n_hyp), dtype=torch.int32, device=dev)
        norm = torch.empty((P, 6), dtype=torch.float32, device=dev)
        F = torch.empty((P, n_hyp, 9), dtype=torch.float32, device=dev) if hyp_F else None
        mk = torch.zeros((P, n_hyp, k_max), dtype=torch.uint8, device=dev) if hyp_mask else None
        prm = RansacParams(int(n_hyp), 0, float(thr), 0, int(seed))
        self._bind_stream()
        _check(self.lib.sfm_ransac_counts(self.handle, _ptr(kps), n_img, k_max, _ptr(pairs), P,
                                          _ptr(count), _ptr(match), C.byref(prm), _ptr(counts),
                                          _ptr(norm), _ptr(F) if hyp_F else None,
                                          _ptr(mk) if hyp_mask else None))
        return (counts, norm, F, mk) if (hyp_F or hyp_mask) else (counts, norm)

    def ransac_h_batch(self, kps, pairs, count, match, n_hyp=4096, seed=42, thr=4.0,
                       min_inliers=15, out=None):
        torch = self.torch
        n_img, k_max, _ = kps.shape
        P = pairs.shape[0]
        dev = kps.device
        if kps.dtype != torch.float32 or not kps.is_contiguous():
            raise SfmCoreError("ransac_h_batch: kps must be contiguous float32")
        if out is None:
            out = dict(inl_count=torch.empty(P, dtype=torch.int32, device=dev),
                       best_h=torch.empty(P, dtype=torch.int32, device=dev),
                       mask=torch.empty((P, k_max), dtype=torch.uint8, device=dev),
                       H=torch.empty((P, 9), dtype=torch.float32, device=dev),
                       norm=torch.empty((P, 6), dtype=torch.float32, device=dev))
        prm = RansacParams(int(n_hyp), int(min_inliers), float(thr), 0, int(seed))
        self._bind_stream()
        _check(self.lib.sfm_ransac_h_batch(self.handle, _ptr(kps), n_img, k_max, _ptr(pairs), P,
                                           _ptr(count), _ptr(match), C.byref(prm),
                                           _ptr(out["inl_count"]), _ptr(out["best_h"]),
                                           _ptr(out["mask"]), _ptr(out["H"]), _ptr(out["norm"])))
        return out

    def ransac_h_counts(self, kps, pairs, count, match, n_hyp=4096, seed=42, thr=4.0,
                        hyp_H=False):
        torch = self.torch
        n_img, k_max, _ = kps.shape
        P = pairs.shape[0]
        dev = kps.device
        if kps.dtype != torch.float32 or not kps.is_contiguous():
            raise SfmCoreError("ransac_h_counts: kps must be contiguous float32")
        counts = torch.empty((P, n_hyp), dtype=torch.int32, device=dev)
        norm = torch.empty((P, 6), dtype=torch.float32, device=dev)
        Hh = torch.empty((P, n_hyp, 9), dtype=torch.float32, device=dev) if hyp_H else None
        prm = RansacParams(int(n_hyp), 0, float(thr), 0, int(seed))
        self._bind_stream()
        _check(self.lib.sfm_ransac_h_counts(self.handle, _ptr(kps), n_img, k_max, _ptr(pairs), P,
                                            _ptr(count), _ptr(match), C.byref(prm), _ptr(counts),
                                            _ptr(norm), _ptr(Hh) if hyp_H else None))
        return (counts, norm, Hh) if hyp_H else (counts, norm)

    def two_view_pose_batch(self, kps, intr, pairs, count, match, mask, inl_count,
                            min_inliers=15, min_angle_deg=2.0, out=None):
        torch = self.torch
        _expect("two_view_pose_batch", ("kps", kps, torch.float32, (kps.shape[1], 2)),
                ("intr", intr, torch.float64, (4,)), ("pairs", pairs, torch.int32, (2,)),
                ("count", count, torch.int32, ()), ("match", match, torch.int32, (kps.shape[1], 2)),
                ("mask", mask, torch.uint8, (kps.shape[1],)),
                ("inl_count", inl_count, torch.int32, ()))
        n_img, k_max, _ = kps.shape
        P = pairs.shape[0]
        if intr.shape[0] != n_img or not (count.shape[0] == match.shape[0] == mask.shape[0]
                                          == inl_count.shape[0] == P):
            raise SfmCoreError("two_view_pose_batch: intr must have one row per image and "
                               "count / match / mask / inl_count one per pair")
        if not 0.0 <= float(min_angle_deg) <= 90.0:
            raise SfmCoreError("two_view_pose_batch: min_angle_deg must lie in [0, 90]")
        dev = kps.device
        if out is None:
            out = dict(E=torch.empty((P, 9), dtype=torch.float64, device=dev),
                       R=torch.empty((P, 9), dtype=torch.float64, device=dev),
                       t=torch.empty((P, 3), dtype=torch.float64, device=dev),
                       stat=torch.empty((P, 8), dtype=torch.int32, device=dev),
                       median_key=torch.empty(P, dtype=torch.float32, device=dev))
        prm = TwoViewPoseParams(C.sizeof(TwoViewPoseParams), int(min_inliers),
                                float(angle_key(min_angle_deg)))
        self._bind_stream()
        _check(self.lib.sfm_two_view_pose_batch(
            self.handle, _ptr(kps), n_img, k_max, _ptr(pairs), P, _ptr(count), _ptr(match),
            _ptr(mask), _ptr(inl_count), _ptr(intr), C.byref(prm), _ptr(out["E"]), _ptr(out["R"]),
            _ptr(out["t"]), _ptr(out["stat"]), _ptr(out["median_key"])))
        return out

    def ransac_stats(self, enable=True, read=False):
        out = (C.c_uint64 * 3)()
        self._bind_stream()
        _check(self.lib.sfm_ransac_stats(self.handle, 1 if enable else 0, out if read else None))
        return (int(out[0]), int(out[1]), int(out[2])) if read else None

    def match_cert_stats(self, enable=True, read=False):
        out = (C.c_uint64 * 3)()
        self._bind_stream()
        _check(self.lib.sfm_match_cert_stats(self.handle, 1 if enable else 0,
                                             out if read else None))
        return (int(out[0]), int(out[1]), int(out[2])) if read else None

    def ransac_wave_stops(self, n_pairs, n_hyp):
        out = np.zeros((n_pairs, n_hyp // 64), np.uint32)
        self._bind_stream()
        _check(self.lib.sfm_ransac_wave_stops(self.handle, int(n_pairs), int(n_hyp),
                                              out.ctypes.data_as(C.c_void_p)))
        return out

    def calib_mfma_i8(self, target_ms=200.0):
        out = np.zeros(4, np.float64)
        self._bind_stream()
        _check(self.lib.sfm_calib_mfma_i8(self.handle, float(target_ms),
                                          out.ctypes.data_as(C.c_void_p)))
        return {"ms": float(out[0]), "tops": float(out[1]), "clock_ghz": float(out[2]),
                "frac_nominal": float(out[3])}

    def graph_rows(self, pair_base, count, match, inl_count, mask, min_inliers=15,
                   return_offsets=False, packed=False):
        torch = self.torch
        P, k_max = mask.shape
        dev = mask.device
        offs = torch.empty(P + 1, dtype=torch.int64, device=dev)
        self._bind_stream()
        _check(self.lib.sfm_graph_offsets(self.handle, P, _ptr(inl_count), int(min_inliers),
                                          _ptr(offs)))
        n = int(offs[P].item())
        rows = torch.empty((n,) if packed else (n, 3), dtype=torch.int32, device=dev)
        if n and packed:
            _check(self.lib.sfm_graph_rows_packed(self.handle, P, k_max, _ptr(count),
                                                  _ptr(match), _ptr(mask), _ptr(inl_count),
                                                  int(min_inliers), _ptr(offs), _ptr(rows)))
        elif n:
            _check(self.lib.sfm_graph_rows(self.handle, P, k_max, int(pair_base), _ptr(count),
                                           _ptr(match), _ptr(mask), _ptr(inl_count),
                                           int(min_inliers), _ptr(offs), _ptr(rows)))
        return (rows, offs) if return_offsets else rows

    def graph_expand(self, pair_base, counts, src_offsets, dst_offsets, packed, n_rows):
        torch = self.torch
        dev = packed.device
        rows = torch.empty((n_rows, 3), dtype=torch.int32, device=dev)
        P = counts.shape[0]
        if P and n_rows:
            self._bind_stream()
            _check(self.lib.sfm_graph_expand(self.handle, P, int(pair_base), _ptr(counts),
                                             _ptr(src_offsets), _ptr(dst_offsets), _ptr(packed),
                                             _ptr(rows)))
        return rows

    def ba_set_chunks(self, spec=None):
        if spec is None:
            _check(self.lib.sfm_ba_set_chunks(self.handle, 0, None, None, 0, None))
            return
        args = getattr(spec, "_cargs", None)
        if args is None:
            n = len(spec.chunk_pt) - 1
            args = spec._cargs = (n, (C.c_int32 * (n + 1))(*[int(v) for v in spec.chunk_pt]),
                                  (C.c_int32 * (n + 1))(*[int(v) for v in spec.chunk_obs]),
                                  int(spec.n_total), _ptr(spec.cam_bounds))
        _check(self.lib.sfm_ba_set_chunks(self.handle, *args))

    def ba_set_schur(self, spec=None):
        if spec is None:
            _check(self.lib.sfm_ba_set_schur(self.handle, 0, None, 0, None, 0, None, None, 0, None,
                                             0, None, None, None))
            return
        _check(self.lib.sfm_ba_set_schur(self.handle, spec.n_slot, _ptr(spec.slot_cam), spec.n_seg,
                                         _ptr(spec.seg), spec.n_inst, _ptr(spec.inst),
                                         _ptr(spec.row_ptr), spec.n_ent, _ptr(spec.row_ent),
                                         spec.n_group, _ptr(spec.sg_ptr), _ptr(spec.sg),
                                         _ptr(spec.gk)))

    def ba_chunk_tree(self, parts, out=None):
        torch = self.torch
        parts = parts.contiguous()
        nt = parts.shape[0]
        if out is None:
            out = torch.empty(parts.shape[1:], dtype=torch.float64, device=parts.device)
        self._bind_stream()
        _check(self.lib.sfm_ba_chunk_tree(self.handle, nt, int(out.numel()), _ptr(parts),
                                          _ptr(out)))
        return out

    def ba_jtj(self, cams, pp, pts, cam_idx, pt_idx, uv, pt_ptr, cam_ptr, cam_obs, loss_s=0.0,
               n_slot=None):
        torch = self.torch
        dev = cams.device
        nc, npt, no = cams.shape[0], pts.shape[0], cam_idx.shape[0]
        f64 = torch.float64
        lead = () if n_slot is None else (n_slot,)
        U = torch.empty(lead + (nc, 8, 8), dtype=f64, device=dev)
        V = torch.empty((npt, 3, 3), dtype=f64, device=dev)
        W = torch.empty((no, 8, 3), dtype=f64, device=dev)
        gc = torch.empty(lead + (nc, 8), dtype=f64, device=dev)
        gp = torch.empty((npt, 3), dtype=f64, device=dev)
        res = torch.empty((no, 2), dtype=f64, device=dev)
        cost = torch.empty(max(n_slot or 1, 1), dtype=f64, device=dev)
        self._bind_stream()
        _check(self.lib.sfm_ba_jtj(self.handle, nc, _ptr(cams), _ptr(pp), npt, _ptr(pts), no,
                                   _ptr(cam_idx), _ptr(pt_idx), _ptr(uv), _ptr(pt_ptr),
                                   _ptr(cam_ptr), _ptr(cam_obs), float(loss_s), _ptr(U), _ptr(V),
                                   _ptr(W), _ptr(gc), _ptr(gp), _ptr(res), _ptr(cost)))
        return dict(U=U, V=V, W=W, gc=gc, gp=gp, res=res, cost=cost)

    def tracks(self, img_base, pairs, rows, min_len=2):
        torch = self.torch
        dev = img_base.device
        n_img = img_base.shape[0] - 1
        n_nodes = int(img_base[-1].item()) if n_img > 0 else 0
        cap = max(n_nodes, 1)
        nt = torch.zeros(1, dtype=torch.int32, device=dev)
        ptr = torch.zeros(cap + 1, dtype=torch.int32, device=dev)
        ti = torch.empty(cap, dtype=torch.int32, device=dev)
        tk = torch.empty(cap, dtype=torch.int32, device=dev)
        self._bind_stream()
        _check(self.lib.sfm_tracks(self.handle, n_img, _ptr(img_base), pairs.shape[0],
                                   _ptr(pairs) if pairs.numel() else None, rows.shape[0],
                                   _ptr(rows) if rows.numel() else None, int(min_len), _ptr(nt),
                                   _ptr(ptr), _ptr(ti), _ptr(tk)))
        T = int(nt.item())
        total = int(ptr[T].item())
        return ptr[:T + 1], ti[:total], tk[:total]

    def register_batch(self, corr_ptr, xy, X, intr, img_id, n_hyp=1024, thr=4.0, seed=42,
                       refine=True):
        torch = self.torch
        dev = xy.device
        n_img = corr_ptr.shape[0] - 1
        n = xy.shape[0]
        _expect("register_batch", ("corr_ptr", corr_ptr, torch.int32, ()),
                ("xy", xy, torch.float64, (2,)), ("X", X, torch.float64, (3,)),
                ("intr", intr, torch.float64, (4,)), ("img_id", img_id, torch.int32, ()))
        if X.shape[0] != n or intr.shape[0] != n_img or img_id.shape[0] != n_img:
            raise SfmCoreError("register_batch: xy / X and intr / img_id / corr_ptr sizes differ")
        cams = torch.empty((max(n_img, 0), 8), dtype=torch.float64, device=dev)
        count = torch.empty(max(n_img, 0), dtype=torch.int32, device=dev)
        key = torch.empty(max(n_img, 0), dtype=torch.int32, device=dev)
        mask = torch.empty(max(n, 1), dtype=torch.uint8, device=dev)
        prm = RegisterParams(int(n_hyp), 1 if refine else 0, float(thr), int(seed))
        self._bind_stream()
        _check(self.lib.sfm_register_batch(self.handle, n_img, _ptr(corr_ptr), _ptr(xy), _ptr(X),
                                           _ptr(intr), _ptr(img_id), C.byref(prm), _ptr(cams),
                                           _ptr(count), _ptr(key), _ptr(mask)))
        return cams, count, key, mask[:n]

    def triangulate(self, cams, pp, pt_ptr, cam_idx, uv):
        torch = self.torch
        n_pt = pt_ptr.shape[0] - 1
        _expect("triangulate", ("cams", cams, torch.float64, (8,)), ("pp", pp, torch.float64, (2,)),
                ("pt_ptr", pt_ptr, torch.int32, ()), ("cam_idx", cam_idx, torch.int32, ()),
                ("uv", uv, torch.float64, (2,)))
        if pp.shape[0] != cams.shape[0] or uv.shape[0] != cam_idx.shape[0]:
            raise SfmCoreError("triangulate: cams / pp or cam_idx / uv sizes differ")
        pts = torch.empty((max(n_pt, 0), 3), dtype=torch.float64, device=cams.device)
        stats = torch.empty((max(n_pt, 0), 4), dtype=torch.float64, device=cams.device)
        self._bind_stream()
        _check(self.lib.sfm_triangulate(self.handle, cams.shape[0], _ptr(cams), _ptr(pp), n_pt,
                                        _ptr(pt_ptr), _ptr(cam_idx), _ptr(uv), _ptr(pts),
                                        _ptr(stats)))
        return pts, stats

    def ba_solve(self, lin, cam_idx, pt_idx, pt_ptr, cam_ptr, cam_obs, lam, max_iter=100,
                 tol=1e-10, out=None, poll=8, poll_first=0):
        torch = self.torch
        U = lin["U"]
        dev = U.device
        nc, npt, no = U.shape[0], lin["V"].shape[0], cam_idx.shape[0]
        if out is None:
            f64 = torch.float64
            out = (torch.empty((nc, 8), dtype=f64, device=dev),
                   torch.empty((npt, 3), dtype=f64, device=dev),
                   torch.empty(5, dtype=f64, device=dev))
        dc, dp, info = out
        prm = BaSolveParams(float(lam), float(tol), int(max_iter), int(poll) if poll > 0 else -1,
                            max(int(poll_first), 0))
        self._bind_stream()
        _check(self.lib.sfm_ba_solve(self.handle, nc, npt, no, _ptr(cam_idx), _ptr(pt_idx),
                                     _ptr(pt_ptr), _ptr(cam_ptr), _ptr(cam_obs), _ptr(U),
                                     _ptr(lin["V"]), _ptr(lin["W"]), _ptr(lin["gc"]),
                                     _ptr(lin["gp"]), C.byref(prm), _ptr(dc), _ptr(dp),
                                     _ptr(info)))
        return dc, dp, info

    def ba_solve_sharded(self, lin, cam_idx, pt_idx, pt_ptr, cam_ptr, cam_obs, lam, allreduce,
                         max_iter=100, tol=1e-10, out=None, poll=8, graph=False, chunks=None,
                         schur=None, poll_first=0):
        torch = self.torch
        U = lin["U"]
        dev = U.device
        nc, npt, no = U.shape[0], lin["V"].shape[0], cam_idx.shape[0]
        if out is None:
            f64 = torch.float64
            out = (torch.empty((nc, 8), dtype=f64, device=dev),
                   torch.empty((npt, 3), dtype=f64, device=dev),
                   torch.empty(5, dtype=f64, device=dev))
        dc, dp, info = out
        nt = chunks.n_total if chunks is not None else 1
        k0 = chunks.k0 if chunks is not None else 0
        ns = schur.n_slot if schur is not None else 0
        n_setup = nt * 44 * nc
        comm = torch.zeros(n_setup + (64 * schur.n_group if ns else 0), dtype=torch.float64,
                           device=dev)
        prm = BaSolveParams(float(lam), float(tol), int(max_iter), int(poll))
        done = C.c_int32(0)
        cptr = comm.data_ptr()

        def args(off=0):
            return (nc, npt, no, _ptr(cam_idx), _ptr(pt_idx), _ptr(pt_ptr), _ptr(cam_ptr),
                    _ptr(cam_obs), _ptr(U), _ptr(lin["V"]), _ptr(lin["W"]), _ptr(lin["gc"]),
                    _ptr(lin["gp"]), C.byref(prm), C.c_void_p(cptr + 8 * off), _ptr(dc), _ptr(dp),
                    _ptr(info), C.byref(done))
        a_base = args()
        a_setup, a_iter, a_back = args(k0 * 44 * nc), args(k0 * 8 * nc), args(k0 * 2)
        self._bind_stream()

        def stage(s, k=0, a=a_base):
            _check(self.lib.sfm_ba_solve_stage(self.handle, s, k, *a))

        def produce(s, n, a, k=0):
            if chunks is not None:
                comm[:n].zero_()
            stage(s, k, a)
            allreduce(comm[:n])
        if ns:
            comm.zero_()
            stage(BA_STAGE_SETUP, 0, a_setup)
            stage(BA_STAGE_SCHUR, 0, args(n_setup + 64 * schur.g0))
            allreduce(comm)
        else:
            produce(BA_STAGE_SETUP, n_setup, a_setup)
        stage(BA_STAGE_SETUP_FINISH)
        every = poll
        graph = (graph and not ns and getattr(allreduce, "graph_safe", False) and every > 0
                 and every % 2 == 0 and nc <= BA_FINISH_VEC_MAX_CAM)
        win = every if every > 0 else max(max_iter, 1)
        win0 = int(poll_first) if every > 0 and poll_first > 0 else win
        g = None
        k = 0
        while k < max_iter:
            if every > 0 and k > 0:
                stage(BA_STAGE_POLL)
                if done.value:
                    break
            n = min(win0 if k == 0 else win, max_iter - k)
            if graph and k > 0 and n == win:
                if g is None:
                    g = torch.cuda.CUDAGraph()
                    cap = torch.cuda.Stream(dev)
                    cap.wait_stream(torch.cuda.current_stream(dev))
                    with torch.cuda.stream(cap):
                        self._bind_stream()
                        g.capture_begin()
                        try:
                            for j in range(n):
                                produce(BA_STAGE_ITER, nt * 8 * nc, a_iter, k + j)
                                stage(BA_STAGE_ITER_FINISH, k + j)
                        finally:
                            g.capture_end()
                    torch.cuda.current_stream(dev).wait_stream(cap)
                    self._bind_stream()
                g.replay()
            elif ns:
                for j in range(k, k + n):
                    stage(BA_STAGE_ITER, j)
            else:
                for j in range(k, k + n):
                    produce(BA_STAGE_ITER, nt * 8 * nc, a_iter, j)
                    stage(BA_STAGE_ITER_FINISH, j)
            k += n
        produce(BA_STAGE_BACKSUB, nt * 2, a_back)
        stage(BA_STAGE_MODEL)
        return dc, dp, info

    def ba_fix_params(self, lin, cam_idx, fixed):
        U = lin["U"]
        nc, no = U.shape[0], cam_idx.shape[0]
        self._bind_stream()
        _check(self.lib.sfm_ba_fix_params(self.handle, nc, no, _ptr(cam_idx), _ptr(fixed),
                                          _ptr(U), _ptr(lin["W"]), _ptr(lin["gc"])))
        return lin

    def ba_cost(self, cams, pp, pts, cam_idx, pt_idx, uv, loss_s=0.0, out=None, n_slot=None):
        torch = self.torch
        cost = out if out is not None else torch.empty(max(n_slot or 1, 1), dtype=torch.float64,
                                                       device=cams.device)
        self._bind_stream()
        _check(self.lib.sfm_ba_cost(self.handle, cams.shape[0], _ptr(cams), _ptr(pp),
                                    pts.shape[0], _ptr(pts), cam_idx.shape[0], _ptr(cam_idx),
                                    _ptr(pt_idx), _ptr(uv), float(loss_s), _ptr(cost)))
        return cost

    def ba_update(self, cams, dc, pts, dp, out=None):
        torch = self.torch
        if out is None:
            out = (torch.empty_like(cams), torch.empty_like(pts))
        co, po = out
        self._bind_stream()
        _check(self.lib.sfm_ba_update(self.handle, cams.shape[0], _ptr(cams), _ptr(dc),
                                      pts.shape[0], _ptr(pts), _ptr(dp), _ptr(co), _ptr(po)))
        return co, po


_ctx_cache: dict = {}


def context(device: int = 0) -> Context:
    ctx = _ctx_cache.get(device)
    if ctx is None:
        ctx = Context(device)
        _ctx_cache[device] = ctx
    return ctx


def csr_by_device(index, n: int):
    import torch
    idx = index.long()
    order = torch.argsort(idx, stable=True).to(torch.int32)
    return csr_ptr_device(idx, n), order


def csr_ptr_device(index, n: int, ascending: bool = False):
    import torch
    idx = index.long()
    dev = index.device
    if ascending:
        return torch.searchsorted(idx, torch.arange(n + 1, dtype=torch.int64, device=dev)).to(torch.int32)
    cnt = torch.zeros(n, dtype=torch.int64, device=dev)
    cnt.index_add_(0, idx, torch.ones_like(idx))
    ptr = torch.zeros(n + 1, dtype=torch.int32, device=dev)
    ptr[1:] = torch.cumsum(cnt, 0).to(torch.int32)
    return ptr


def csr_by(index: np.ndarray, n: int):
    order = np.argsort(index, kind="stable").astype(np.int32)
    ptr = np.zeros(n + 1, np.int32)
    np.cumsum(np.bincount(index, minlength=n), out=ptr[1:])
    return ptr, order
```

Measured before the change: 259.0 million verified matches/s.

## Fuse compact and mutual-cert tails; run reverse scan only on flagged pairs

The separate compact and mutual-certificate kernels are merged into one templated tail kernel. It either writes matches directly or appends uncertified pairs to a flag list. The reverse scan and final kernels become persistent 1024-block grids that walk only the flagged pairs instead of launching over every pair. The setup kernel drops the reverse-order block. This saves a launch and global round-trips of intermediate records, and skips reverse scanning for pairs the certificate already resolves. The cost is a heavier tail kernel (large LDS, launch bounds 3) and a fixed grid size that may underfill or serialize when many pairs are flagged.

```diff
diff --git a/include/sfmcore.h b/include/sfmcore.h
--- a/include/sfmcore.h
+++ b/include/sfmcore.h
@@ -199,6 +199,8 @@
 
 int sfm_match_cert_stats(sfm_ctx* ctx, int32_t enable, uint64_t* out);
 
+int32_t sfm_l2fr_rev_grid(void);
+
 #ifdef __cplusplus
 }
 #endif
diff --git a/sfm-project_amd/csrc/match_l2fr.hip b/sfm-project_amd/csrc/match_l2fr.hip
--- a/sfm-project_amd/csrc/match_l2fr.hip
+++ b/sfm-project_amd/csrc/match_l2fr.hip
@@ -149,7 +149,7 @@
 }
 
 __device__ void order_block(int ob, const int32_t* __restrict__ pairs, int n_pairs, int n_img,
-                            int32_t* __restrict__ order_f, int32_t* __restrict__ order_r,
+                            int32_t* __restrict__ order,
                             int2* __restrict__ rng, int32_t* __restrict__ n_rng,
                             const int32_t* __restrict__ n_kp, int4* __restrict__ rinfo,
                             int4* __restrict__ sinfo_f, int unit_blk, int4* __restrict__ uinfo,
@@ -158,11 +158,10 @@
         build_units(pairs, n_pairs, n_img, n_kp, uinfo, n_units, hist);
         return;
     }
-    const int tid = threadIdx.x, col = ob == 0 ? 1 : 0;
-    int32_t* order = ob == 0 ? order_f : order_r;
+    const int tid = threadIdx.x;
     for (int i = tid; i < n_img; i += 1024) hist[i] = 0;
     __syncthreads();
-    for (int p = tid; p < n_pairs; p += 1024) atomicAdd(&hist[pairs[2 * p + col]], 1);
+    for (int p = tid; p < n_pairs; p += 1024) atomicAdd(&hist[pairs[2 * p + 1]], 1);
     __syncthreads();
     int* roff = hist + n_img;
     if (tid == 0) {
@@ -174,24 +173,22 @@
             hist[i] = off;
             off += c;
         }
-        if (ob == 0) *n_rng = nr;
-    }
-    __syncthreads();
-    if (ob == 0)
-        for (int i = tid; i < n_img; i += 1024) {
-            const int c = (i + 1 < n_img ? hist[i + 1] : n_pairs) - hist[i];
-            for (int k = 0; k < c; k += REC_R)
-                rng[roff[i] + k / REC_R] = make_int2(hist[i] + k, min(REC_R, c - k));
-        }
-    __syncthreads();
+        n_rng[0] = nr;
+        n_rng[1] = 0;
+    }
+    __syncthreads();
+    for (int i = tid; i < n_img; i += 1024) {
+        const int c = (i + 1 < n_img ? hist[i + 1] : n_pairs) - hist[i];
+        for (int k = 0; k < c; k += REC_R)
+            rng[roff[i] + k / REC_R] = make_int2(hist[i] + k, min(REC_R, c - k));
+    }
     __syncthreads();
     for (int p = tid; p < n_pairs; p += 1024) {
         const int a = pairs[2 * p], b = pairs[2 * p + 1];
-        const int slot = atomicAdd(&hist[col ? b : a], 1);
+        const int slot = atomicAdd(&hist[b], 1);
         order[slot] = p;
-        if (ob == 0) sinfo_f[slot] = make_int4(p, a, b, n_kp[a] | (n_kp[b] << 16));
-    }
-    if (ob != 0) return;
+        sinfo_f[slot] = make_int4(p, a, b, n_kp[a] | (n_kp[b] << 16));
+    }
     __threadfence_block();
     __syncthreads();
     const int nr = *n_rng;
@@ -213,7 +210,7 @@
     int n_prep, int bpi, const uint8_t* __restrict__ desc, const int32_t* __restrict__ n_kp,
     int k_max, int k_pad, int32_t* __restrict__ norm, int32_t* __restrict__ cinit,
     uint8_t* __restrict__ zero_row, uint4* __restrict__ desc_i8, const int32_t* __restrict__ pairs,
-    int n_pairs, int n_img, int32_t* __restrict__ order_f, int32_t* __restrict__ order_r,
+    int n_pairs, int n_img, int32_t* __restrict__ order_f,
     int2* __restrict__ rng, int32_t* __restrict__ n_rng, int4* __restrict__ rinfo,
     int4* __restrict__ sinfo_f, int unit_blk, int4* __restrict__ uinfo,
     int32_t* __restrict__ n_units) {
@@ -225,7 +222,7 @@
                  cinit, zero_row, desc_i8);
         return;
     }
-    order_block(b - n_prep, pairs, n_pairs, n_img, order_f, order_r, rng, n_rng, n_kp, rinfo,
+    order_block(b - n_prep, pairs, n_pairs, n_img, order_f, rng, n_rng, n_kp, rinfo,
                 sinfo_f, unit_blk, uinfo, n_units, hist);
 }
 
@@ -251,13 +248,14 @@
 constexpr int L2FR_CLOCK_W = 24;
 __device__ unsigned long long g_l2fr_clock[L2FR_CLOCK_W * L2FR_CLOCK_SLOTS];
 #define L2FR_STAMP(i, v) \
-    if (!REV && tid == 0 && blockIdx.x < L2FR_CLOCK_SLOTS) g_l2fr_clock[L2FR_CLOCK_W * (size_t)blockIdx.x + (i)] = (v)
+    if (!REV && tid == 0 && bid < L2FR_CLOCK_SLOTS) g_l2fr_clock[L2FR_CLOCK_W * (size_t)bid + (i)] = (v)
 #else
 #define L2FR_STAMP(i, v)
 #endif
 
 template <bool REV>
-__global__ __launch_bounds__(SCAN_THREADS, SCAN_MIN_WAVES) void l2fr_scan_kernel(
+__device__ __forceinline__ void scan_body(
+    const unsigned bid, const unsigned n_bid, const int n_list,
     const uint8_t* __restrict__ desc, const int32_t* __restrict__ n_kp, int k_max, int k_pad,
     const int32_t* __restrict__ cinit, const uint8_t* __restrict__ zero_row,
     const int32_t* __restrict__ pairs, int n_qblk, const int32_t* __restrict__ pair_order,
@@ -273,9 +271,9 @@
     if (!REV && n_units) {
         const int nu = *n_units;
         const int u8 = (nu + 7) >> 3;
-        const int l = (int)(blockIdx.x >> 3);
+        const int l = (int)(bid >> 3);
         qb = u8 > 0 ? l / u8 : n_qblk;
-        pos = (l - qb * u8) * 8 + (int)(blockIdx.x & 7);
+        pos = (l - qb * u8) * 8 + (int)(bid & 7);
         if (qb >= n_qblk || pos >= nu) return;
         const int4 u = sinfo[(size_t)UNIT * pos];
         asm volatile("" : : "s"(u.x), "s"(u.y), "s"(u.z), "s"(u.w));
@@ -284,27 +282,26 @@
         ti = u.z;
         nq = u.w & 0xFFFF;
         nb = u.w >> 16;
+    } else if (REV) {
+        qb = (int)bid / n_list;
+        p = pair_order[(int)bid - qb * n_list];
+        qi = pairs[2 * p + 1];
+        ti = pairs[2 * p];
+        nq = qcount[p];
+        nb = n_kp[ti];
     } else {
-        const int ppx = (int)(gridDim.x >> 3) / n_qblk;
-        const int l = (int)(blockIdx.x >> 3);
-        const int pos = (int)(blockIdx.x & 7) * ppx + l % ppx;
+        const int ppx = (int)(n_bid >> 3) / n_qblk;
+        const int l = (int)(bid >> 3);
+        const int pos = (int)(bid & 7) * ppx + l % ppx;
         qb = l / ppx;
         if (pos >= n_blk) return;
-        if (REV) {
-            p = pair_order[pos];
-            qi = pairs[2 * p + 1];
-            ti = pairs[2 * p];
-            nq = qcount[p];
-            nb = n_kp[ti];
-        } else {
-            const int4 u = sinfo[pos];
-            asm volatile("" : : "s"(u.x), "s"(u.y), "s"(u.z), "s"(u.w));
-            p = u.x;
-            qi = u.y;
-            ti = u.z;
-            nq = u.w & 0xFFFF;
-            nb = u.w >> 16;
-        }
+        const int4 u = sinfo[pos];
+        asm volatile("" : : "s"(u.x), "s"(u.y), "s"(u.z), "s"(u.w));
+        p = u.x;
+        qi = u.y;
+        ti = u.z;
+        nq = u.w & 0xFFFF;
+        nb = u.w >> 16;
     }
     if (qb * QB >= nq || nb <= 0) return;
     const int tid = threadIdx.x, wave = tid >> 6, lane = tid & 63, h = lane >> 5, r32 = lane & 31;
@@ -591,6 +588,30 @@
 #endif
 }
 
+__global__ __launch_bounds__(SCAN_THREADS, SCAN_MIN_WAVES) void l2fr_scan_fwd_kernel(
+    const uint8_t* __restrict__ desc, const int32_t* __restrict__ n_kp, int k_max, int k_pad,
+    const int32_t* __restrict__ cinit, const uint8_t* __restrict__ zero_row,
+    const int32_t* __restrict__ pairs, int n_qblk, const int4* __restrict__ sinfo, int n_blk,
+    FwdCls fc, const int32_t* __restrict__ n_units) {
+    scan_body<false>(blockIdx.x, gridDim.x, 0, desc, n_kp, k_max, k_pad, cinit, zero_row, pairs, n_qblk,
+                     nullptr, sinfo, n_blk, nullptr, nullptr, nullptr, fc, n_units);
+}
+
+constexpr int REV_GRID = 1024;
+__global__ __launch_bounds__(SCAN_THREADS, SCAN_MIN_WAVES) void l2fr_scan_rev_kernel(
+    const uint8_t* __restrict__ desc, const int32_t* __restrict__ n_kp, int k_max, int k_pad,
+    const int32_t* __restrict__ cinit, const uint8_t* __restrict__ zero_row,
+    const int32_t* __restrict__ pairs, int n_qblk, const int32_t* __restrict__ flist,
+    const int32_t* __restrict__ n_flag, const int4* __restrict__ qlist,
+    const int32_t* __restrict__ qcount, int4* __restrict__ out) {
+    const int nl = *n_flag;
+    for (unsigned u = blockIdx.x; u < (unsigned)(nl * n_qblk); u += gridDim.x) {
+        scan_body<true>(u, 0, nl, desc, n_kp, k_max, k_pad, cinit, zero_row, pairs, n_qblk, flist,
+                        nullptr, 0, qlist, qcount, out, FwdCls{}, nullptr);
+        __syncthreads();
+    }
+}
+
 struct Top2 { long long b1; int j1; long long b2; };
 
 __device__ __forceinline__ Top2 top2_merge(Top2 x, Top2 y) {
@@ -839,202 +860,275 @@
     }
 }
 
-__global__ __launch_bounds__(256) void l2fr_compact_kernel(
+constexpr int CERT_TMAX = 2048;
+constexpr long long CERT_CAP_DEFAULT = 16384;
+constexpr int TAIL_NQ = KMAX / 256;
+enum : int { TAIL_DIRECT = 0, TAIL_CERT = 1, TAIL_SPILL = 2 };
+
+template <int MODE>
+__global__ __launch_bounds__(256, 3) void l2fr_tail_kernel(
     const uint8_t* __restrict__ desc, const int32_t* __restrict__ n_kp, int k_max, int k_pad,
     const int32_t* __restrict__ norm, const int32_t* __restrict__ pairs,
-    const uint8_t* __restrict__ cls, rec8* __restrict__ qst, int rnum, int rden, long long max_dist,
-    int4* __restrict__ surv, int32_t* __restrict__ scount, int32_t* __restrict__ smax,
-    int32_t* __restrict__ out_count, int32_t* __restrict__ out_match,
-    int32_t* __restrict__ out_dist) {
-    __shared__ Top2 red[256];
-    __shared__ int slow[256];
-    __shared__ int nslow, wsum[8], wmax[4];
-    const int p = blockIdx.x, tid = threadIdx.x;
+    const rec8* __restrict__ fwd, const uint8_t* __restrict__ cls, rec8* qst, int rnum, int rden,
+    long long max_dist, long long cap, int4* surv, int32_t* __restrict__ scount,
+    int32_t* __restrict__ flist, int32_t* __restrict__ n_flag,
+    unsigned long long* __restrict__ stats, int32_t* __restrict__ out_count,
+    int32_t* __restrict__ out_match, int32_t* __restrict__ out_dist) {
+    __shared__ unsigned long long owner[KMAX];
+    __shared__ int tbound[CERT_TMAX];
+    __shared__ unsigned short tq[CERT_TMAX];
+    __shared__ unsigned char killed[KMAX];
+    __shared__ __attribute__((aligned(16))) int wcnt[TAIL_NQ][4];
+    __shared__ int wmax[4];
+    __shared__ int nthreat, nslow;
+    Top2* red = (Top2*)owner;
+    unsigned short* slowq = (unsigned short*)(owner + 1024);
+    static_assert(sizeof(Top2) * 256 <= 8192, "the row scan's slots overlap the slow list");
+    const int p = blockIdx.x, tid = threadIdx.x, lane = tid & 63, wave = tid >> 6;
     const int a = pairs[2 * p], b = pairs[2 * p + 1];
     const int na = n_kp[a], nb = n_kp[b];
-    const bool direct = out_count != nullptr;
-    int32_t* om = direct ? out_match + (size_t)p * k_max * 2 : nullptr;
-    int32_t* od = direct ? out_dist + (size_t)p * k_max : nullptr;
     if (na <= 0 || nb <= 0) {
         if (tid == 0) {
-            if (direct) out_count[p] = 0;
-            else scount[p] = 0;
+            if (MODE == TAIL_SPILL || (MODE == TAIL_CERT && cap <= 0)) {
+                scount[p] = 0;
+                flist[atomicAdd(n_flag, 1)] = p;
+                if (MODE == TAIL_CERT && stats) atomicAdd(&stats[1], 1ull);
+            } else {
+                out_count[p] = 0;
+                if (MODE == TAIL_CERT && stats) atomicAdd(&stats[0], 1ull);
+            }
         }
         return;
     }
+    const int nq = na;
     rec8* qs = qst + (size_t)p * k_pad;
+    const rec8* fw = fwd + (size_t)p * k_pad;
     const uint8_t* cl = cls + (size_t)p * k_pad;
     const int32_t* na_norm = norm + (size_t)a * k_pad;
     const int32_t* nb_norm = norm + (size_t)b * k_pad;
     const uint4* qa = (const uint4*)(desc + (size_t)a * k_max * D);
-    const uint8_t* db = desc + (size_t)b * k_max * D;
+    const uint4* dbv = (const uint4*)(desc + (size_t)b * k_max * D);
     int4* sv = surv + (size_t)p * k_pad;
-    int base = 0, dmax = 0;
-    for (int q0 = 0; q0 < na; q0 += 256) {
-        const int q = q0 + tid;
-        int4 r = make_int4(ST_DROP, 0, 0, 0);
-        if (q < na) {
-            const unsigned char c = cl[q];
-            const rec8 raw = qs[q];
-            if (c == l2fr::CLS_SLOW) {
-                r.x = ST_SLOW;
-            } else if (c != l2fr::CLS_DROP) {
-                const l2fr::Res u = l2fr::unpack_res(raw);
-                r = make_int4(u.st, u.j1, u.d1, u.exact);
-            }
-        }
-        if (tid == 0) nslow = 0;
-        __syncthreads();
-        if (r.x == ST_SLOW) slow[atomicAdd(&nslow, 1)] = tid;
+    int32_t* om = out_match + (size_t)p * k_max * 2;
+    int32_t* od = out_dist + (size_t)p * k_max;
+
+    rec8 raw[TAIL_NQ];
+    int bnd[TAIL_NQ];
+    unsigned hasm = 0, slowm = 0;
+#pragma unroll
+    for (int i0 = 0; i0 < TAIL_NQ; i0 += TAIL_NQ / 2) {
+        if (i0 * 256 >= nq) {
+#pragma unroll
+            for (int i = i0; i < i0 + TAIL_NQ / 2; ++i) {
+                raw[i] = 0;
+                bnd[i] = INT_MAX;
+            }
+            continue;
+        }
+        unsigned char c[TAIL_NQ / 2];
+        rec8 fr[TAIL_NQ / 2];
+        int A[TAIL_NQ / 2];
+#pragma unroll
+        for (int k = 0; k < TAIL_NQ / 2; ++k) {
+            const int qc = min((i0 + k) * 256 + tid, nq - 1);
+            c[k] = cl[qc];
+            raw[i0 + k] = qs[qc];
+            if (MODE == TAIL_CERT) {
+                fr[k] = fw[qc];
+                A[k] = na_norm[qc];
+            }
+        }
+#pragma unroll
+        for (int k = 0; k < TAIL_NQ / 2; ++k) {
+            const int i = i0 + k;
+            const bool in = i * 256 + tid < nq;
+            const bool has = in && c[k] != l2fr::CLS_DROP;
+            const bool slow =
+                in && (c[k] == l2fr::CLS_SLOW || (has && l2fr::unpack_res(raw[i]).st == ST_SLOW));
+            hasm |= has ? 1u << i : 0u;
+            slowm |= slow ? 1u << i : 0u;
+            bnd[i] = INT_MAX;
+            if (MODE == TAIL_CERT) {
+                const l2fr::Fwd f = l2fr::unpack_fwd(fr[k]);
+                const int known = f.e2 > E_VALID ? A[k] - 2 * f.e2 - 1 : INT_MAX;
+                bnd[i] = !in ? INT_MAX : (has ? known : A[k] - 2 * f.e1 - 1);
+            }
+        }
+    }
+    if (tid == 0) nslow = 0;
+    if (__syncthreads_or(slowm != 0)) {
+#pragma unroll
+        for (int i = 0; i < TAIL_NQ; ++i)
+            if ((slowm >> i) & 1u) slowq[atomicAdd(&nslow, 1)] = (unsigned short)(i * 256 + tid);
         __syncthreads();
         const int ns = nslow;
-        for (int i = 0; i < ns; ++i) {
-            const int who = slow[i], qq = q0 + who;
-            const Top2 e = exact_row_scan(qa + (size_t)qq * SLOTS, db, nb_norm, nb, na_norm[qq], red);
-            if (tid == who) {
+        for (int k = 0; k < ns; ++k) {
+            const int qq = slowq[k];
+            const Top2 e = exact_row_scan(qa + (size_t)qq * SLOTS, (const uint8_t*)dbv, nb_norm, nb,
+                                          na_norm[qq], red);
+            if (tid == (qq & 255)) {
                 bool keep = sfm::ratio_ok(e.b1, e.b2, rnum, rden, true);
                 keep = keep && (max_dist < 0 || e.b1 < max_dist);
-                r = make_int4(keep ? ST_PASS : ST_DROP, e.j1, (int)e.b1, 1);
-                if (!direct) qs[qq] = l2fr::pack_res(r.x, r.y, r.z, 1);
-            }
-        }
-        const bool keep = r.x == ST_PASS;
-        dmax = keep ? max(dmax, r.z) : dmax;
-        if (direct)
-            base = sfm::compact256(keep, q, r.y, r.z, base, wsum, om, od);
-        else
-            base = compact_rec(keep, make_int4(q, r.y, r.z, 0), base, wsum, sv);
-    }
-    if (tid == 0) {
-        if (direct) out_count[p] = base;
-        else scount[p] = base;
-    }
-    if (direct) return;
+                qs[qq] = l2fr::pack_res(keep ? ST_PASS : ST_DROP, e.j1, (int)e.b1, 1);
+            }
+        }
+        __syncthreads();
+#pragma unroll
+        for (int i = 0; i < TAIL_NQ; ++i)
+            if ((slowm >> i) & 1u) raw[i] = qs[i * 256 + tid];
+    }
+    unsigned keepm = 0;
+    int dmax = 0;
+#pragma unroll
+    for (int i = 0; i < TAIL_NQ; ++i) {
+        const l2fr::Res r = l2fr::unpack_res(raw[i]);
+        const bool keep = ((hasm >> i) & 1u) && r.st == ST_PASS;
+        keepm |= keep ? 1u << i : 0u;
+        dmax = keep ? max(dmax, r.d1) : dmax;
+        const unsigned long long bal = __ballot(keep);
+        if (lane == 0) wcnt[i][wave] = __popcll(bal);
+    }
 #pragma unroll
     for (int m = 32; m > 0; m >>= 1) dmax = max(dmax, __shfl_xor(dmax, m));
-    if ((tid & 63) == 0) wmax[tid >> 6] = dmax;
-    __syncthreads();
-    if (tid == 0) smax[p] = max(max(wmax[0], wmax[1]), max(wmax[2], wmax[3]));
-}
-
-constexpr int CERT_TMAX = 2048;
-constexpr long long CERT_CAP_DEFAULT = 16384;
-
-__global__ __launch_bounds__(256) void l2fr_mutual_cert_kernel(
-    const uint8_t* __restrict__ desc, const int32_t* __restrict__ n_kp, int k_max, int k_pad,
-    const int32_t* __restrict__ norm, const int32_t* __restrict__ pairs,
-    const rec8* __restrict__ fwd, const uint8_t* __restrict__ cls, const rec8* __restrict__ qst,
-    const int4* __restrict__ surv, const int32_t* __restrict__ scount,
-    const int32_t* __restrict__ smax, long long cap, int32_t* __restrict__ rcount,
-    uint8_t* __restrict__ flag, unsigned long long* __restrict__ stats,
-    int32_t* __restrict__ out_count, int32_t* __restrict__ out_match,
-    int32_t* __restrict__ out_dist) {
-    __shared__ unsigned long long owner[KMAX];
-    __shared__ int tbound[CERT_TMAX];
-    __shared__ unsigned short tq[CERT_TMAX];
-    __shared__ unsigned char killed[KMAX];
-    __shared__ int wsum[8];
-    __shared__ int nthreat;
-    const int p = blockIdx.x, tid = threadIdx.x;
-    const int a = pairs[2 * p], b = pairs[2 * p + 1];
-    const int na = n_kp[a], nb = n_kp[b];
-    const int S = (na > 0 && nb > 0) ? scount[p] : 0;
-    if (cap <= 0) {
+    if (lane == 0) wmax[wave] = dmax;
+    if (MODE == TAIL_CERT) {
+        for (int k = tid; k < nq; k += 256) killed[k] = 0;
+        for (int j = tid; j < nb; j += 256) owner[j] = ~0ull;
+        if (tid == 0) nthreat = 0;
+    }
+    __syncthreads();
+    unsigned slot2[TAIL_NQ / 2] = {};
+    auto slot = [&](int i) { return (int)((slot2[i >> 1] >> (16 * (i & 1))) & 0xFFFFu); };
+    int S = 0;
+#pragma unroll
+    for (int i = 0; i < TAIL_NQ; ++i) {
+        const int4 w4 = *(const int4*)wcnt[i];
+        const int ww[4] = {w4.x, w4.y, w4.z, w4.w};
+        int off = S;
+#pragma unroll
+        for (int w = 0; w < 4; ++w) {
+            off += w < wave ? ww[w] : 0;
+            S += ww[w];
+        }
+        const unsigned long long bal = __ballot((keepm >> i) & 1u);
+        slot2[i >> 1] |= (unsigned)(off + __popcll(bal & ((1ull << lane) - 1ull))) << (16 * (i & 1));
+    }
+    const int T = max(max(wmax[0], wmax[1]), max(wmax[2], wmax[3]));
+
+    if (MODE == TAIL_DIRECT) {
+#pragma unroll
+        for (int i = 0; i < TAIL_NQ; ++i)
+            if ((keepm >> i) & 1u) {
+                const l2fr::Res r = l2fr::unpack_res(raw[i]);
+                om[2 * slot(i)] = i * 256 + tid;
+                om[2 * slot(i) + 1] = r.j1;
+                od[slot(i)] = r.d1;
+            }
+        if (tid == 0) out_count[p] = S;
+        return;
+    }
+    auto spill = [&]() {
+#pragma unroll
+        for (int i = 0; i < TAIL_NQ; ++i)
+            if ((keepm >> i) & 1u) {
+                const l2fr::Res r = l2fr::unpack_res(raw[i]);
+                sv[slot(i)] = make_int4(i * 256 + tid, r.j1, r.d1, 0);
+            }
+    };
+    auto flag_pair = [&]() {
+        spill();
         if (tid == 0) {
-            rcount[p] = S;
-            flag[p] = 1;
-            if (stats) atomicAdd(&stats[1], 1ull);
-        }
+            scount[p] = S;
+            flist[atomicAdd(n_flag, 1)] = p;
+            if (MODE == TAIL_CERT && stats) atomicAdd(&stats[1], 1ull);
+        }
+    };
+    if (MODE == TAIL_SPILL || cap <= 0) {
+        flag_pair();
         return;
     }
     if (S == 0) {
         if (tid == 0) {
-            rcount[p] = 0;
-            flag[p] = 0;
             out_count[p] = 0;
             if (stats) atomicAdd(&stats[0], 1ull);
         }
         return;
     }
-    const rec8* fw = fwd + (size_t)p * k_pad;
-    const rec8* qs = qst + (size_t)p * k_pad;
-    const uint8_t* cl = cls + (size_t)p * k_pad;
-    const int4* sv = surv + (size_t)p * k_pad;
-    const int32_t* na_norm = norm + (size_t)a * k_pad;
-    const int32_t* nb_norm = norm + (size_t)b * k_pad;
-    const uint4* qa = (const uint4*)(desc + (size_t)a * k_max * D);
-    const uint4* dbv = (const uint4*)(desc + (size_t)b * k_max * D);
-
-    const long long T = smax[p];
-    for (int k = tid; k < S; k += 256) killed[k] = 0;
-    for (int j = tid; j < nb; j += 256) owner[j] = ~0ull;
-    if (tid == 0) nthreat = 0;
-    __syncthreads();
-
-    for (int q = tid; q < na; q += 256) {
-        const unsigned char c = cl[q];
-        const rec8 raw = qs[q];
-        l2fr::Res r{ST_DROP, 0, 0, 0};
-        if (c != l2fr::CLS_DROP) r = l2fr::unpack_res(raw);
-        const l2fr::Fwd f = l2fr::unpack_fwd(fw[q]);
-        const long long A = na_norm[q];
-        long long bound;
-        if (r.exact == 1) {
+#pragma unroll
+    for (int i = 0; i < TAIL_NQ; ++i) {
+        const int q = i * 256 + tid;
+        if ((hasm >> i) & 1u) {
+            const l2fr::Res r = l2fr::unpack_res(raw[i]);
             if ((unsigned)r.j1 < (unsigned)nb)
                 atomicMin(&owner[r.j1], ((unsigned long long)(unsigned)r.d1 << 32) | (unsigned)q);
-            bound = f.e2 > E_VALID ? A - 2LL * f.e2 - 1 : sfm::DIST_INF;
-        } else {
-            bound = A - 2LL * f.e1 - 1;
-        }
-        if (bound <= T) {
-            const int i = atomicAdd(&nthreat, 1);
-            if (i < CERT_TMAX) {
-                tq[i] = (unsigned short)q;
-                tbound[i] = (int)bound;
+        }
+        if (bnd[i] <= T) {
+            const int k = atomicAdd(&nthreat, 1);
+            if (k < CERT_TMAX) {
+                tq[k] = (unsigned short)q;
+                tbound[k] = bnd[i];
             }
         }
     }
     __syncthreads();
     const int nT = nthreat;
     if (nT > CERT_TMAX || (long long)nT * S > cap) {
-        if (tid == 0) {
-            rcount[p] = S;
-            flag[p] = 1;
-            if (stats) atomicAdd(&stats[1], 1ull);
-        }
+        flag_pair();
         return;
     }
-    unsigned dots = 0;
-    for (int i = tid; i < nT * S; i += 256) {
-        const int t = i / S, k = i - t * S;
-        const int4 s = sv[k];
-        const int qp = tq[t];
-        if (qp == s.x || s.z < tbound[t]) continue;
-        const int dot = dot128(qa + (size_t)qp * SLOTS, dbv + (size_t)s.y * SLOTS);
-        const long long d = (long long)na_norm[qp] + nb_norm[s.y] - 2LL * dot;
-        if (d < s.z || (d == s.z && qp < s.x)) killed[k] = 1;
-        ++dots;
-    }
-    if (stats && dots) atomicAdd(&stats[2], (unsigned long long)dots);
-    __syncthreads();
-    int32_t* om = out_match + (size_t)p * k_max * 2;
-    int32_t* od = out_dist + (size_t)p * k_max;
-    int base = 0;
-    for (int k0 = 0; k0 < S; k0 += 256) {
-        const int k = k0 + tid;
-        int4 s = make_int4(0, 0, 0, 0);
+    if (nT > 0) {
+        spill();
+        __syncthreads();
+        unsigned dots = 0;
+        for (int i = tid; i < nT * S; i += 256) {
+            const int t = i / S, k = i - t * S;
+            const int4 s = sv[k];
+            const int qp = tq[t];
+            if (qp == s.x || s.z < tbound[t]) continue;
+            const int dot = dot128(qa + (size_t)qp * SLOTS, dbv + (size_t)s.y * SLOTS);
+            const long long d = (long long)na_norm[qp] + nb_norm[s.y] - 2LL * dot;
+            if (d < s.z || (d == s.z && qp < s.x)) killed[k] = 1;
+            ++dots;
+        }
+        if (stats && dots) atomicAdd(&stats[2], (unsigned long long)dots);
+        __syncthreads();
+    }
+    unsigned outm = 0;
+#pragma unroll
+    for (int i = 0; i < TAIL_NQ; ++i) {
         bool keep = false;
-        if (k < S) {
-            s = sv[k];
-            keep = !killed[k] &&
-                   owner[s.y] == (((unsigned long long)(unsigned)s.z << 32) | (unsigned)s.x);
-        }
-        base = sfm::compact256(keep, s.x, s.y, s.z, base, wsum, om, od);
+        if ((keepm >> i) & 1u) {
+            const l2fr::Res r = l2fr::unpack_res(raw[i]);
+            keep = !killed[slot(i)] &&
+                   owner[r.j1] == (((unsigned long long)(unsigned)r.d1 << 32) | (unsigned)(i * 256 + tid));
+        }
+        outm |= keep ? 1u << i : 0u;
+        const unsigned long long bal = __ballot(keep);
+        if (lane == 0) wcnt[i][wave] = __popcll(bal);
+    }
+    __syncthreads();
+    int M = 0;
+#pragma unroll
+    for (int i = 0; i < TAIL_NQ; ++i) {
+        const int4 w4 = *(const int4*)wcnt[i];
+        const int ww[4] = {w4.x, w4.y, w4.z, w4.w};
+        int off = M;
+#pragma unroll
+        for (int w = 0; w < 4; ++w) {
+            off += w < wave ? ww[w] : 0;
+            M += ww[w];
+        }
+        const unsigned long long bal = __ballot((outm >> i) & 1u);
+        if ((outm >> i) & 1u) {
+            const int o = off + __popcll(bal & ((1ull << lane) - 1ull));
+            const l2fr::Res r = l2fr::unpack_res(raw[i]);
+            om[2 * o] = i * 256 + tid;
+            om[2 * o + 1] = r.j1;
+            od[o] = r.d1;
+        }
     }
     if (tid == 0) {
-        out_count[p] = base;
-        rcount[p] = 0;
-        flag[p] = 0;
+        out_count[p] = M;
         if (stats) atomicAdd(&stats[0], 1ull);
     }
 }
@@ -1043,20 +1137,22 @@
     const uint8_t* __restrict__ desc, const int32_t* __restrict__ n_kp, int k_max, int k_pad,
     const int32_t* __restrict__ norm, const int32_t* __restrict__ cinit,
     const int32_t* __restrict__ pairs, const int4* __restrict__ surv,
-    const int32_t* __restrict__ scount, const int4* __restrict__ rev, int mutual,
-    const uint8_t* __restrict__ flag, int32_t* __restrict__ out_count,
-    int32_t* __restrict__ out_match, int32_t* __restrict__ out_dist) {
+    const int32_t* __restrict__ scount, const int4* __restrict__ rev,
+    const int32_t* __restrict__ flist, const int32_t* __restrict__ n_flag,
+    int32_t* __restrict__ out_count, int32_t* __restrict__ out_match,
+    int32_t* __restrict__ out_dist) {
     __shared__ int wsum[8];
     __shared__ int amb[256];
     __shared__ int namb;
     __shared__ unsigned char keepx[256];
     __shared__ long long redd[256];
     __shared__ int redq[256];
-    const int p = blockIdx.x, tid = threadIdx.x;
-    if (flag && !flag[p]) return;
+    const int tid = threadIdx.x, nl = *n_flag;
+    for (int li = blockIdx.x; li < nl; li += gridDim.x) {
+    const int p = flist[li];
     const int a = pairs[2 * p], b = pairs[2 * p + 1];
-    const int na = n_kp[a], nb = n_kp[b];
-    const int S = (na > 0 && nb > 0) ? scount[p] : 0;
+    const int na = n_kp[a];
+    const int S = scount[p];
     const int4* sv = surv + (size_t)p * k_pad;
     const int4* rv = rev + (size_t)p * k_pad;
     const int32_t* na_norm = norm + (size_t)a * k_pad;
@@ -1075,14 +1171,11 @@
         __syncthreads();
         if (k < S) {
             s = sv[k];
-            keep = true;
-            if (mutual) {
-                const int4 r = rv[k];
-                const int dot = (int)(((long long)na_norm[s.x] + nb_norm[s.y] - s.z) >> 1);
-                const int ep = dot + ca[s.x];
-                keep = (ep == r.x) && (r.y < r.x);
-                if (ep == r.x && r.y == r.x) amb[atomicAdd(&namb, 1)] = tid;
-            }
+            const int4 r = rv[k];
+            const int dot = (int)(((long long)na_norm[s.x] + nb_norm[s.y] - s.z) >> 1);
+            const int ep = dot + ca[s.x];
+            keep = (ep == r.x) && (r.y < r.x);
+            if (ep == r.x && r.y == r.x) amb[atomicAdd(&namb, 1)] = tid;
         }
         keepx[tid] = keep;
         __syncthreads();
@@ -1119,6 +1212,7 @@
         base = sfm::compact256(keep, s.x, s.y, s.z, base, wsum, om, od);
     }
     if (tid == 0) out_count[p] = base;
+    }
 }
 
 __global__ void l2fr_dump_kernel(const int32_t* __restrict__ n_kp, const int32_t* __restrict__ pairs,
@@ -1168,10 +1262,9 @@
     const size_t rinfob = sizeof(int4) * (size_t)n_rng_max * REC_R;
     const size_t sinfob = sfm::align_up(sizeof(int4) * (size_t)n_pairs, 256);
     const size_t uinfob = sfm::align_up(UNIT * sizeof(int4) * (size_t)n_pairs, 256);
-    const size_t flagb = sfm::align_up((size_t)n_pairs, 256);
-    char* ws = (char*)sfm::workspace(ctx, 256 + 2 * tab + 2 * recb + cntb + descb + 2 * ordb + clsb +
+    char* ws = (char*)sfm::workspace(ctx, 256 + 2 * tab + 2 * recb + cntb + descb + ordb + clsb +
                                               256 + rngb + rinfob + 256 + sinfob + uinfob + 256 +
-                                              cntb + flagb + cntb);
+                                              cntb);
     if (!ws) return SFM_ERR_NOMEM;
     char* w = ws;
     uint8_t* zero_row = (uint8_t*)w; w += 256;
@@ -1184,17 +1277,15 @@
     int32_t* scount = (int32_t*)w; w += cntb;
     uint8_t* desc_i8 = (uint8_t*)w; w += descb;
     int32_t* ord_f = (int32_t*)w; w += ordb;
-    int32_t* ord_r = (int32_t*)w; w += ordb;
     uint8_t* cls = (uint8_t*)w; w += clsb;
     int32_t* n_rng = (int32_t*)w; w += 256;
+    int32_t* n_flag = n_rng + 1;
     int2* rng = (int2*)w; w += rngb;
     int4* rinfo = (int4*)w; w += rinfob;
     int4* sinfo_f = (int4*)sfm::align_up((size_t)w, 256);
     int4* uinfo = (int4*)((char*)sinfo_f + sinfob);
     int32_t* n_units = (int32_t*)((char*)uinfo + uinfob);
-    int32_t* rcount = (int32_t*)((char*)n_units + 256);
-    uint8_t* flag = (uint8_t*)rcount + cntb;
-    int32_t* smax = (int32_t*)(flag + flagb);
+    int32_t* flist = (int32_t*)((char*)n_units + 256);
     static const bool units_env = [] {
         const char* e = getenv("SFM_L2FR_UNITS");
         return !(e && e[0] == '0');
@@ -1205,25 +1296,21 @@
     const int grid = 8 * ppx * n_qblk;
     const bool mutual = prm->cross_check == SFM_XC_MUTUAL;
 
-    const int32_t* sord_f = ord_f;
-    const int32_t* sord_r = ord_r;
-    const int unit_blk = units ? (mutual ? 2 : 1) : -1;
+    const int unit_blk = units ? 1 : -1;
     const int bpi = (k_pad + 1023) / 1024, n_prep = bpi * n_img;
-    hipLaunchKernelGGL(l2fr_setup_kernel, dim3(n_prep + (mutual ? 2 : 1) + (units ? 1 : 0)),
-                       dim3(1024), ((units ? 3 : 2) * (size_t)n_img + 2) * sizeof(int), st, n_prep,
-                       bpi, desc, n_kp, k_max, k_pad, norm, cinit, zero_row, (uint4*)desc_i8, pairs,
-                       n_pairs, n_img, ord_f, ord_r, rng, n_rng, rinfo, sinfo_f, unit_blk, uinfo,
-                       n_units);
+    hipLaunchKernelGGL(l2fr_setup_kernel, dim3(n_prep + 1 + (units ? 1 : 0)), dim3(1024),
+                       ((units ? 3 : 2) * (size_t)n_img + 2) * sizeof(int), st, n_prep, bpi, desc, n_kp,
+                       k_max, k_pad, norm, cinit, zero_row, (uint4*)desc_i8, pairs, n_pairs, n_img,
+                       ord_f, rng, n_rng, rinfo, sinfo_f, unit_blk, uinfo, n_units);
     SFM_HIP_CHECK(hipGetLastError());
     const FwdCls fc{norm, prm->ratio_num, prm->ratio_den, (long long)prm->max_dist, fwd, cls};
-    hipLaunchKernelGGL(l2fr_scan_kernel<false>, dim3(grid), dim3(SCAN_THREADS), 0, st, desc_i8, n_kp, k_max,
-                       k_pad, cinit, zero_row, pairs, n_qblk, sord_f,
-                       (const int4*)(units ? uinfo : sinfo_f), n_blk, (const int4*)nullptr,
-                       (const int32_t*)nullptr, (int4*)nullptr, fc,
-                       (const int32_t*)(units ? n_units : nullptr));
+    hipLaunchKernelGGL(l2fr_scan_fwd_kernel, dim3(grid), dim3(SCAN_THREADS), 0, st, desc_i8, n_kp, k_max,
+                       k_pad, cinit, zero_row, pairs, n_qblk, (const int4*)(units ? uinfo : sinfo_f),
+                       n_blk, fc, (const int32_t*)(units ? n_units : nullptr));
     SFM_HIP_CHECK(hipGetLastError());
     const char* dbg = getenv("SFM_L2FR_DEBUG");
-    const int dmode = dbg ? atoi(dbg) : 0;
+    int dmode = dbg ? atoi(dbg) : 0;
+    if (dmode < 1 || dmode > 3) dmode = 0;
     if (dmode == 1) {
         hipLaunchKernelGGL(l2fr_dump_kernel, dim3(n_pairs), dim3(256), 0, st, n_kp, pairs, k_max,
                            k_pad, (const int4*)nullptr, (const rec8*)fwd, (const int32_t*)nullptr,
@@ -1235,41 +1322,32 @@
                        (const rec8*)fwd, (const uint8_t*)cls, prm->ratio_num, prm->ratio_den,
                        (long long)prm->max_dist, qst);
     SFM_HIP_CHECK(hipGetLastError());
-    const bool direct = !mutual && dmode == 0;
-    hipLaunchKernelGGL(l2fr_compact_kernel, dim3(n_pairs), dim3(256), 0, st, desc_i8, n_kp, k_max,
-                       k_pad, norm, pairs, (const uint8_t*)cls, qst, prm->ratio_num, prm->ratio_den,
-                       (long long)prm->max_dist, surv, scount, smax,
-                       direct ? out_count : nullptr,
+    const char* ce = getenv("SFM_L2FR_CERT");
+    const bool cert = mutual && dmode == 0 && !(ce && ce[0] == '0');
+    const char* cc = getenv("SFM_L2FR_CERT_CAP");
+    const long long cap = cc ? atoll(cc) : CERT_CAP_DEFAULT;
+    unsigned long long* stats = cert && ctx->cert_stats ? ctx->cert_acc : nullptr;
+    if (stats)
+        SFM_HIP_CHECK(hipMemsetAsync(stats, 0, 3 * sizeof(unsigned long long), st));
+    auto tail = !mutual && dmode == 0 ? l2fr_tail_kernel<TAIL_DIRECT>
+                : cert                ? l2fr_tail_kernel<TAIL_CERT>
+                                      : l2fr_tail_kernel<TAIL_SPILL>;
+    hipLaunchKernelGGL(tail, dim3(n_pairs), dim3(256), 0, st, desc_i8, n_kp, k_max, k_pad, norm, pairs,
+                       (const rec8*)fwd, (const uint8_t*)cls, qst, prm->ratio_num, prm->ratio_den,
+                       (long long)prm->max_dist, cap, surv, scount, flist, n_flag, stats, out_count,
                        out_match, out_dist);
     SFM_HIP_CHECK(hipGetLastError());
-    if (direct) return SFM_OK;
+    if (!mutual && dmode == 0) return SFM_OK;
     if (dmode == 2) {
         hipLaunchKernelGGL(l2fr_dump_kernel, dim3(n_pairs), dim3(256), 0, st, n_kp, pairs, k_max,
                            k_pad, (const int4*)surv, (const rec8*)nullptr, (const int32_t*)scount,
                            out_count, out_match, out_dist);
         return SFM_OK;
     }
-    const char* ce = getenv("SFM_L2FR_CERT");
-    const bool cert = mutual && dmode == 0 && !(ce && ce[0] == '0');
-    if (cert) {
-        const char* cc = getenv("SFM_L2FR_CERT_CAP");
-        const long long cap = cc ? atoll(cc) : CERT_CAP_DEFAULT;
-        unsigned long long* stats = ctx->cert_stats ? ctx->cert_acc : nullptr;
-        if (stats)
-            SFM_HIP_CHECK(hipMemsetAsync(stats, 0, 3 * sizeof(unsigned long long), st));
-        hipLaunchKernelGGL(l2fr_mutual_cert_kernel, dim3(n_pairs), dim3(256), 0, st, desc_i8, n_kp,
-                           k_max, k_pad, norm, pairs, (const rec8*)fwd, (const uint8_t*)cls,
-                           (const rec8*)qst, (const int4*)surv, (const int32_t*)scount,
-                           (const int32_t*)smax, cap, rcount, flag, stats,
-                           out_count, out_match, out_dist);
-        SFM_HIP_CHECK(hipGetLastError());
-    }
     if (mutual) {
-        hipLaunchKernelGGL(l2fr_scan_kernel<true>, dim3(grid), dim3(SCAN_THREADS), 0, st, desc_i8, n_kp,
-                           k_max, k_pad, cinit, zero_row, pairs, n_qblk, sord_r,
-                           (const int4*)nullptr, n_blk,
-                           (const int4*)surv, (const int32_t*)(cert ? rcount : scount), rev, fc,
-                           (const int32_t*)nullptr);
+        hipLaunchKernelGGL(l2fr_scan_rev_kernel, dim3(REV_GRID), dim3(SCAN_THREADS), 0, st, desc_i8, n_kp,
+                           k_max, k_pad, cinit, zero_row, pairs, n_qblk, (const int32_t*)flist,
+                           (const int32_t*)n_flag, (const int4*)surv, (const int32_t*)scount, rev);
         SFM_HIP_CHECK(hipGetLastError());
     }
     if (dmode == 3) {
@@ -1278,12 +1356,14 @@
                            out_count, out_match, out_dist);
         return SFM_OK;
     }
-    hipLaunchKernelGGL(l2fr_final_kernel, dim3(n_pairs), dim3(256), 0, st, desc_i8, n_kp, k_max,
-                       k_pad, norm, cinit, pairs, surv, scount, rev, mutual ? 1 : 0,
-                       (const uint8_t*)(cert ? flag : nullptr), out_count, out_match, out_dist);
+    hipLaunchKernelGGL(l2fr_final_kernel, dim3(REV_GRID), dim3(256), 0, st, desc_i8, n_kp, k_max, k_pad,
+                       norm, cinit, pairs, surv, scount, rev, (const int32_t*)flist,
+                       (const int32_t*)n_flag, out_count, out_match, out_dist);
     SFM_HIP_CHECK(hipGetLastError());
     return SFM_OK;
 }
+
+extern "C" int32_t sfm_l2fr_rev_grid(void) { return REV_GRID; }
 
 extern "C" int sfm_match_cert_stats(sfm_ctx* ctx, int32_t enable, uint64_t* out) {
     SFM_REQUIRE(ctx, "sfm_match_cert_stats: ctx is NULL");
diff --git a/sfm-project_amd/sfmcore.py b/sfm-project_amd/sfmcore.py
--- a/sfm-project_amd/sfmcore.py
+++ b/sfm-project_amd/sfmcore.py
@@ -21,7 +21,7 @@
             "sfm_graph_expand", "sfm_match_batch_both", "sfm_ransac_wave_stops",
             "sfm_ba_set_chunks", "sfm_ba_chunk_tree", "sfm_ba_set_schur", "sfm_calib_mfma_i8",
             "sfm_match_cert_stats", "sfm_ransac_h_batch", "sfm_ransac_h_counts",
-            "sfm_two_view_pose_batch"]
+            "sfm_two_view_pose_batch", "sfm_l2fr_rev_grid"]
 
 
 class SfmCoreError(RuntimeError):
@@ -101,6 +101,8 @@
         L.sfm_ransac_stats.argtypes = [vp, i32, vp]
         L.sfm_ransac_wave_stops.argtypes = [vp, i32, i32, vp]
         L.sfm_match_cert_stats.argtypes = [vp, i32, vp]
+        L.sfm_l2fr_rev_grid.argtypes = []
+        L.sfm_l2fr_rev_grid.restype = i32
         L.sfm_calib_mfma_i8.argtypes = [vp, C.c_float, vp]
         L.sfm_ba_jtj.argtypes = [vp, i32, vp, vp, i32, vp, i32, vp, vp, vp, vp, vp, vp, f64, vp,
                                  vp, vp, vp, vp, vp, vp]
@@ -375,6 +377,9 @@
         _check(self.lib.sfm_match_cert_stats(self.handle, 1 if enable else 0,
                                              out if read else None))
         return (int(out[0]), int(out[1]), int(out[2])) if read else None
+
+    def l2fr_rev_grid(self):
+        return int(self.lib.sfm_l2fr_rev_grid())
 
     def ransac_wave_stops(self, n_pairs, n_hyp):
         out = np.zeros((n_pairs, n_hyp // 64), np.uint32)
```

Measured after the change: 263.7 million verified matches/s (median of 6 runs). 1.8% higher.
